# USTC3DV/D3Human-code

Measured on AMD Instinct MI355X. Metric: train iters/sec @ tet-res 128, 1024^2 render; 1/2/4/8 MI355X, higher is better.
Workload: dtype f32

## Files before the change

d3human-code_amd/csrc/sdf_mlp_bwd.hip:

```cpp
#include "sdf_mlp_dev.h"
#include "sdf_mlp_x3.h"
#include <type_traits>

using namespace D3H_MLP_NS;

namespace {

__global__ void sdf_mlp_pack_t_kernel(const float* __restrict__ w0, const float* __restrict__ wh, const float* __restrict__ w4,
                                      float* __restrict__ wpackT) {
    int idx = blockIdx.x * blockDim.x + threadIdx.x;
    if (idx >= WPACKT_FLOATS) return;
    int l = t_layer_of_offset(idx);
    int local = idx - t_layer_offset(l);
    int r = local & 3, lane = (local >> 2) & 63, rest = local >> 8;
    int i = lane & 15, q = lane >> 4;
    int blk = rest & 15, rbg = rest >> 4;
    int out = 16 * blk + 4 * q + r;
    int in = 16 * rbg + i;
    float v = 0.f;
    if (l == 0) {
        if (in < EMB_DIM) v = w0[out * EMB_DIM + in];
    } else if (l == 4) {
        if (rbg < 16) v = w4[out * (256 + EMB_DIM) + in];
        else {
            int e = in - 256;
            if (e < EMB_DIM) v = w4[out * (256 + EMB_DIM) + 256 + e];
        }
    } else {
        int hi = (l < 4) ? (l - 1) : (l - 2);
        v = wh[(size_t)hi * 65536 + out * 256 + in];
    }
    wpackT[idx] = v;
}

__global__ __launch_bounds__(256) void sdf_mlp_active_tiles_kernel(const float* __restrict__ gout, int64_t n, int ntiles16, int* __restrict__ list,
                                                                   int* __restrict__ count) {
    int t = blockIdx.x * 256 + threadIdx.x;
    bool act = false;
    if (t < ntiles16) {
        int64_t p0 = (int64_t)t * 16;
#pragma unroll
        for (int k = 0; k < 16; ++k)
            if (p0 + k < n) {
#pragma unroll
                for (int o = 0; o < NOUT; ++o)
                    if (gout[(p0 + k) * NOUT + o] != 0.f) act = true;
            }
    }
    unsigned long long m = __ballot(act);
    int lane = threadIdx.x & 63;
    int base = 0;
    if (lane == 0 && m) base = atomicAdd(count, __popcll(m));
    base = __shfl(base, 0);
    if (act) list[base + __popcll(m & ((1ull << lane) - 1ull))] = t;
}

#if D3H_MLP_NOUT == 1
__global__ __launch_bounds__(256) void sdf_mlp_active_points_kernel(const float* __restrict__ gout, int64_t n, int* __restrict__ plist, int* __restrict__ counts) {
    const int64_t p = (int64_t)blockIdx.x * 256 + threadIdx.x;
    const float gv = p < n ? gout[p] : 0.f;
    const bool act = p < n && gv != 0.f;
    {
        float m = fabsf(gv);
        if (!(m < 3.0e38f)) m = 0.f;
#pragma unroll
        for (int k = 32; k > 0; k >>= 1) m = fmaxf(m, __shfl_xor(m, k));
        if ((threadIdx.x & 63) == 0 && m > 0.f) atomicMax((unsigned*)counts + 2, __float_as_uint(m));
    }
    const unsigned long long m = __ballot(act);
    const int lane = threadIdx.x & 63;
    int base = 0;
    if (lane == 0 && m) base = atomicAdd(counts, __popcll(m));
    base = __shfl(base, 0);
    if (act) plist[base + __popcll(m & ((1ull << lane) - 1ull))] = (int)p;
}
__global__ __launch_bounds__(256) void sdf_mlp_gather_points_kernel(const float* __restrict__ x, const float* __restrict__ deform, float disp,
                                                                    const float* __restrict__ gout, const int* __restrict__ plist, int* __restrict__ counts,
                                                                    int* __restrict__ ident, float* __restrict__ xg, float* __restrict__ gg) {
    const int cnt = counts[0];
    const int ntile = (cnt + 15) >> 4;
    if (blockIdx.x == 0 && threadIdx.x == 0) counts[1] = ntile;
    for (int g = blockIdx.x * 256 + threadIdx.x; g < ntile * 16; g += gridDim.x * 256) {
        float x0 = 0.f, x1 = 0.f, x2 = 0.f, gv = 0.f;
        if (g < cnt) {
            const int64_t p = plist[g];
            x0 = x[3 * p + 0]; x1 = x[3 * p + 1]; x2 = x[3 * p + 2];
            if (deform) {
                x0 = __fadd_rn(x0, __fmul_rn(disp, deform[3 * p + 0]));
                x1 = __fadd_rn(x1, __fmul_rn(disp, deform[3 * p + 1]));
                x2 = __fadd_rn(x2, __fmul_rn(disp, deform[3 * p + 2]));
            }
            gv = gout[p];
        }
        xg[3 * (size_t)g + 0] = x0; xg[3 * (size_t)g + 1] = x1; xg[3 * (size_t)g + 2] = x2;
        gg[g] = gv;
        if ((g & 15) == 0) ident[g >> 4] = g >> 4;
    }
}
__global__ __launch_bounds__(256) void sdf_mlp_gather_gout_kernel(const float* __restrict__ gout, const int* __restrict__ plist, int* __restrict__ counts,
                                                                  float* __restrict__ gg) {
    const int cnt = counts[0];
    const int ntile = (cnt + 15) >> 4;
    float m = 0.f;
    for (int g = blockIdx.x * 256 + threadIdx.x; g < ntile * 16; g += gridDim.x * 256) {
        const float gv = g < cnt ? gout[plist[g]] : 0.f;
        gg[g] = gv;
        const float a = fabsf(gv);
        if (a < 3.0e38f) m = fmaxf(m, a);
    }
#pragma unroll
    for (int k = 32; k > 0; k >>= 1) m = fmaxf(m, __shfl_xor(m, k));
    if ((threadIdx.x & 63) == 0 && m > 0.f) atomicMax((unsigned*)counts + 6, __float_as_uint(m));
}
__global__ __launch_bounds__(256) void sdf_mlp_scatter_dx_kernel(const float* __restrict__ dxg, const int* __restrict__ plist, const int* __restrict__ counts,
                                                                 float* __restrict__ dx) {
    const int cnt = counts[0];
    for (int g = blockIdx.x * 256 + threadIdx.x; g < cnt; g += gridDim.x * 256) {
        const int64_t p = plist[g];
        dx[3 * p + 0] = dxg[3 * (size_t)g + 0]; dx[3 * p + 1] = dxg[3 * (size_t)g + 1]; dx[3 * p + 2] = dxg[3 * (size_t)g + 2];
    }
}
#endif

__device__ __forceinline__ void dz_block(f32x4& v, const float* act_l, float* dz_l, int rb, int lane) {
    size_t off = (size_t)(rb * 64 + lane) * 4;
    f32x4 hh = *(const f32x4*)(act_l + off);
    f32x4 o;
#pragma unroll
    for (int r = 0; r < 4; ++r) {
        o[r] = v[r] * dsoftplus_from_h(hh[r]);
        v[r] = o[r];
    }
    *(f32x4*)(dz_l + off) = o;
}

__device__ __forceinline__ void dz_block_inject(f32x4& v, const float* act_l, float* e_l, int rb, int lane) {
    size_t off = (size_t)(rb * 64 + lane) * 4;
    f32x4 hh = *(const f32x4*)(act_l + off);
    f32x4 ee = *(const f32x4*)(e_l + off);
    f32x4 o;
#pragma unroll
    for (int r = 0; r < 4; ++r) {
        o[r] = v[r] * dsoftplus_from_h(hh[r]) + ee[r];
        v[r] = o[r];
    }
    *(f32x4*)(e_l + off) = o;
}

__device__ __forceinline__ void dz_block_pre(f32x4& v, const f32x4 hh, float* dz_l, int rb, int lane) {
    f32x4 o;
#pragma unroll
    for (int r = 0; r < 4; ++r) {
        o[r] = v[r] * dsoftplus_from_h(hh[r]);
        v[r] = o[r];
    }
    *(f32x4*)(dz_l + (size_t)(rb * 64 + lane) * 4) = o;
}
__device__ __forceinline__ void dz_block_inject_pre(f32x4& v, const f32x4 hh, const f32x4 ee, float* e_l, int rb, int lane) {
    f32x4 o;
#pragma unroll
    for (int r = 0; r < 4; ++r) {
        o[r] = v[r] * dsoftplus_from_h(hh[r]) + ee[r];
        v[r] = o[r];
    }
    *(f32x4*)(e_l + (size_t)(rb * 64 + lane) * 4) = o;
}


template <bool INJECT>
__global__ __launch_bounds__(NTHREADS, 2) void sdf_mlp_bwd_data_kernel(const float* __restrict__ x, const float* __restrict__ deform, float disp,
                                                                      const float* __restrict__ gout, const float* __restrict__ w7,
                                                                      const float* __restrict__ wpackT, const float* __restrict__ act,
                                                                      float* __restrict__ dz, float* __restrict__ dx, int64_t n, int ntiles,
                                                                      const int* __restrict__ tile_list, const int* __restrict__ tile_count) {
    __shared__ __attribute__((aligned(16))) float wbuf[2][T_CHUNK_FLOATS];
    __shared__ __attribute__((aligned(16))) float w7s[NOUT * 256];
    __shared__ __attribute__((aligned(16))) float pfb[NWAVES * (INJECT ? 4 : 2) * 256];
    const int n_active = tile_list ? *tile_count : 0;
    const int64_t n16 = tile_list ? (int64_t)n_active : (int64_t)ntiles * 8;
    const int G = (int)gridDim.x;
    const int nrounds = (int)((n16 + NWAVES * (int64_t)G - 1) / (NWAVES * (int64_t)G));

    const int tid = threadIdx.x;
    const int lane = tid & 63;
    const int wave = tid >> 6;
    const int q = lane >> 4;
    constexpr int N4 = T_CHUNK_FLOATS / 4;

    for (int j = tid; j < NOUT * 256; j += NTHREADS) w7s[j] = w7[j];
    Stage st;
    int pb = 0;
    SDF_STAGE_ISSUE(st, wpackT, wbuf[0], N4, tid);
    SDF_STAGE_COMMIT(st, wbuf[0], N4, tid);

    f32x4 X[16], Y[16];
#if D3H_SDF_PRIO
    if (wave >= 4) __builtin_amdgcn_s_setprio(1);
#endif

    for (int rnd = 0; rnd < nrounds; ++rnd) {
        const int64_t seq = (int64_t)rnd * NWAVES * G + (int64_t)wave * G + blockIdx.x;
        const bool on = seq < n16;
        const int64_t t16 = on ? (tile_list ? (int64_t)tile_list[seq] : seq) : 0;
        const int64_t p = t16 * 16 + (lane & 15);
        const bool valid = on && p < n;
        const float* act_tile = act + t16 * ACT_TILE_FLOATS;
        float* dz_tile = dz + t16 * ACT_TILE_FLOATS;
        float g[NOUT];
#pragma unroll
        for (int o = 0; o < NOUT; ++o) g[o] = INJECT ? 0.f : (valid ? (gout ? gout[p * NOUT + o] : 1.f) : 0.f);

#pragma unroll
        for (int rb = 0; rb < 16; ++rb) {
            X[rb] = (f32x4){0.f, 0.f, 0.f, 0.f};
#pragma unroll
            for (int o = 0; o < NOUT; ++o) {
                f32x4 w = *(const f32x4*)(w7s + 256 * o + 16 * rb + 4 * q);
#pragma unroll
                for (int r = 0; r < 4; ++r) X[rb][r] = fmaf(g[o], w[r], X[rb][r]);
            }
        }

        f32x4 E[EMB_BLKS];
#pragma unroll
        for (int b = 0; b < EMB_BLKS; ++b) E[b] = (f32x4){0.f, 0.f, 0.f, 0.f};

        float* pf = pfb + wave * ((INJECT ? 4 : 2) * 256);
        auto prefetch = [&](int lp, int c) {
            const size_t o0 = (size_t)lp * ACT_LAYER_FLOATS + (size_t)((2 * c) * 64 + lane) * 4;
            D3H_GLDS16(act_tile + o0, pf);
            D3H_GLDS16(act_tile + o0 + 256, pf + 256);
            if (INJECT) {
                D3H_GLDS16(dz_tile + o0, pf + 512);
                D3H_GLDS16(dz_tile + o0 + 256, pf + 768);
            }
        };
        auto dz_pair = [&](f32x4& v0, f32x4& v1, int lp, int c) {
            const float* pl = pf + lane * 4;
            float* dzl = dz_tile + lp * ACT_LAYER_FLOATS;
            if (INJECT) {
                dz_block_inject_pre(v0, *(const f32x4*)pl, *(const f32x4*)(pl + 512), dzl, 2 * c, lane);
                dz_block_inject_pre(v1, *(const f32x4*)(pl + 256), *(const f32x4*)(pl + 768), dzl, 2 * c + 1, lane);
            } else {
                dz_block_pre(v0, *(const f32x4*)pl, dzl, 2 * c, lane);
                dz_block_pre(v1, *(const f32x4*)(pl + 256), dzl, 2 * c + 1, lane);
            }
        };
        const float* next = wpackT + T_CHUNK_FLOATS;
        for (int it = 0; it < 3; ++it) {
            {
                const int l = 6 - 2 * it;
                if (on && it == 0) {
#pragma unroll
                    for (int rb = 0; rb < 16; ++rb) {
                        if (INJECT) dz_block_inject(X[rb], act_tile + l * ACT_LAYER_FLOATS, dz_tile + l * ACT_LAYER_FLOATS, rb, lane);
                        else dz_block(X[rb], act_tile + l * ACT_LAYER_FLOATS, dz_tile + l * ACT_LAYER_FLOATS, rb, lane);
                    }
                }
#pragma unroll
                for (int c = 0; c < 8; ++c) {
                    SDF_STAGE_ISSUE(st, next, wbuf[pb ^ 1], N4, tid);
                    next += T_CHUNK_FLOATS;
                    if (on) prefetch(l - 1, c);
                    if (on) {
                        f32x4 acc0 = {0.f, 0.f, 0.f, 0.f}, acc1 = {0.f, 0.f, 0.f, 0.f};
                        mac_hidden2(acc0, acc1, X, wbuf[pb], 16 * 256, lane);
                        Y[2 * c] = acc0;
                        Y[2 * c + 1] = acc1;
                    }
                    __builtin_amdgcn_s_waitcnt(0x0f70);
                    SDF_STAGE_COMMIT(st, wbuf[pb ^ 1], N4, tid);
                    pb ^= 1;
                    if (on) dz_pair(Y[2 * c], Y[2 * c + 1], l - 1, c);
                }
                if (l == 4) {
#pragma unroll
                    for (int c = 0; c < 2; ++c) {
                        SDF_STAGE_ISSUE(st, next, wbuf[pb ^ 1], N4, tid);
                        next += T_CHUNK_FLOATS;
                        if (on) {
                            mac_hidden(E[2 * c], X, wbuf[pb], lane);
                            if (2 * c + 1 < EMB_BLKS) mac_hidden(E[2 * c + 1], X, wbuf[pb] + 16 * 256, lane);
                        }
                        SDF_STAGE_COMMIT(st, wbuf[pb ^ 1], N4, tid);
                        pb ^= 1;
                    }
                }
            }
            {
                const int l = 5 - 2 * it;
#pragma unroll
                for (int c = 0; c < 8; ++c) {
                    SDF_STAGE_ISSUE(st, next, wbuf[pb ^ 1], N4, tid);
                    next += T_CHUNK_FLOATS;
                    if (on) prefetch(l - 1, c);
                    if (on) {
                        f32x4 acc0 = {0.f, 0.f, 0.f, 0.f}, acc1 = {0.f, 0.f, 0.f, 0.f};
                        mac_hidden2(acc0, acc1, Y, wbuf[pb], 16 * 256, lane);
                        X[2 * c] = acc0;
                        X[2 * c + 1] = acc1;
                    }
                    __builtin_amdgcn_s_waitcnt(0x0f70);
                    SDF_STAGE_COMMIT(st, wbuf[pb ^ 1], N4, tid);
                    pb ^= 1;
                    if (on) dz_pair(X[2 * c], X[2 * c + 1], l - 1, c);
                }
            }
        }
#pragma unroll
        for (int c = 0; c < 2; ++c) {
            SDF_STAGE_ISSUE(st, (c == 0) ? next : wpackT, wbuf[pb ^ 1], N4, tid);
            next += T_CHUNK_FLOATS;
            if (on) {
                mac_hidden(E[2 * c], X, wbuf[pb], lane);
                if (2 * c + 1 < EMB_BLKS) mac_hidden(E[2 * c + 1], X, wbuf[pb] + 16 * 256, lane);
            }
            SDF_STAGE_COMMIT(st, wbuf[pb ^ 1], N4, tid);
            pb ^= 1;
        }

        if (!INJECT && dx && on) {
            float x0 = 0.f, x1 = 0.f, x2 = 0.f;
            if (valid) {
                x0 = x[3 * p + 0]; x1 = x[3 * p + 1]; x2 = x[3 * p + 2];
                if (deform) {
                    x0 = __fadd_rn(x0, __fmul_rn(disp, deform[3 * p + 0]));
                    x1 = __fadd_rn(x1, __fmul_rn(disp, deform[3 * p + 1]));
                    x2 = __fadd_rn(x2, __fmul_rn(disp, deform[3 * p + 2]));
                }
            }
            float d0 = 0.f, d1 = 0.f, d2 = 0.f;
#pragma unroll
            for (int b = 0; b < EMB_BLKS; ++b)
#pragma unroll
                for (int r = 0; r < 4; ++r) {
                    int e = 16 * b + 4 * q + r;
                    if (e < EMB_DIM) {
                        float ge = E[b][r];
                        int c;
                        float coef;
                        if (e < 3) { c = e; coef = 1.f; }
                        else {
                            int ep = e - 3;
                            int fr = ep / 6, fn = (ep % 6) / 3;
                            c = ep % 3;
                            float f = (float)(1 << fr);
                            float xc = c == 0 ? x0 : (c == 1 ? x1 : x2);
                            coef = fn ? (-f * sinf(f * xc)) : (f * cosf(f * xc));
                        }
                        float t = ge * coef;
                        if (c == 0) d0 += t; else if (c == 1) d1 += t; else d2 += t;
                    }
                }
            d0 += __shfl_xor(d0, 16); d0 += __shfl_xor(d0, 32);
            d1 += __shfl_xor(d1, 16); d1 += __shfl_xor(d1, 32);
            d2 += __shfl_xor(d2, 16); d2 += __shfl_xor(d2, 32);
            if (valid && q == 0) { dx[3 * p + 0] = d0; dx[3 * p + 1] = d1; dx[3 * p + 2] = d2; }
        }
    }
#if D3H_SDF_GLDS
    __builtin_amdgcn_s_waitcnt(0x0f70);
#endif
}

#if D3H_MLP_NOUT == 1
template <int NP>
__global__ void sdf_mlp_pack_t3_kernel(const float* __restrict__ w0, const float* __restrict__ wh, const float* __restrict__ w4,
                                       unsigned* __restrict__ wpackT3) {
    int idx = blockIdx.x * blockDim.x + threadIdx.x;
    if (idx >= XPT<NP>::WPACKT_DWORDS) return;
    const int chunk = idx / XPT<NP>::HID_CHUNK;
    const int l = t_layer_of_offset(chunk * T_CHUNK_FLOATS);
    const int local = idx - (t_layer_offset(l) / T_CHUNK_FLOATS) * XPT<NP>::HID_CHUNK;
    const int d = local & 3, lane = (local >> 2) & 63;
    int rest = local >> 8;
    const int part = rest % NP;
    rest /= NP;
    const int kb = rest & 7, rbg = rest >> 3;
    const int i = lane & 15, q = lane >> 4;
    const int in = 16 * rbg + i;
    unsigned bits[2];
#pragma unroll
    for (int e = 0; e < 2; ++e) {
        const int out = x3_feature(kb, q, 2 * d + e);
        float v = 0.f;
        if (l == 0) {
            if (in < EMB_DIM) v = w0[out * EMB_DIM + in];
        } else if (l == 4) {
            if (rbg < 16) v = w4[out * (256 + EMB_DIM) + in];
            else if (in - 256 < EMB_DIM) v = w4[out * (256 + EMB_DIM) + in];
        } else {
            const int hi = (l < 4) ? (l - 1) : (l - 2);
            v = wh[(size_t)hi * 65536 + out * 256 + in];
        }
        unsigned h, m, lo = 0;
        if constexpr (NP == 3) x3_split_pair(v, 0.f, h, m, lo);
        else {
            h2_split_pair(v, 0.f, h, m);
            if (!(fabsf(v) <= 16384.0f)) h = m = 0x7e00u;
        }
        bits[e] = (part == 0 ? h : (part == 1 ? m : lo)) & 0xffffu;
    }
    wpackT3[idx] = bits[0] | (bits[1] << 16);
}

__global__ __launch_bounds__(256) void h2_scale_from_absmax_kernel(const float* __restrict__ v, int64_t n, const unsigned* __restrict__ bits, float* __restrict__ sc) {
    __shared__ float red[256];
    float m = 0.f;
    if (bits) m = __uint_as_float(*bits);
    else
        for (int64_t i = threadIdx.x; i < n; i += 256) m = fmaxf(m, fabsf(v[i]));
    red[threadIdx.x] = m;
    __syncthreads();
    for (int k = 128; k > 0; k >>= 1) {
        if ((int)threadIdx.x < k) red[threadIdx.x] = fmaxf(red[threadIdx.x], red[threadIdx.x + k]);
        __syncthreads();
    }
    if (threadIdx.x == 0) {
        const float s = h2_grad_scale(red[0]);
        sc[0] = s;
        sc[1] = 1.0f / s;
    }
}

template <bool SCALED>
__device__ __forceinline__ void dzs_plain(f32x4& v, const f32x4 hh, float* dz_l, int rb, int lane, float gsi) {
    f32x4 o;
#pragma unroll
    for (int r = 0; r < 4; ++r) {
        v[r] = v[r] * dsoftplus_from_h(hh[r]);
        o[r] = SCALED ? v[r] * gsi : v[r];
    }
    *(f32x4*)(dz_l + (size_t)(rb * 64 + lane) * 4) = o;
}
template <bool SCALED>
__device__ __forceinline__ void dzs_inject(f32x4& v, const f32x4 hh, const f32x4 ee, float* e_l, int rb, int lane, float gs, float gsi) {
    f32x4 o;
#pragma unroll
    for (int r = 0; r < 4; ++r) {
        v[r] = SCALED ? fmaf(ee[r], gs, v[r] * dsoftplus_from_h(hh[r])) : (v[r] * dsoftplus_from_h(hh[r]) + ee[r]);
        o[r] = SCALED ? v[r] * gsi : v[r];
    }
    *(f32x4*)(e_l + (size_t)(rb * 64 + lane) * 4) = o;
}

template <bool INJECT, int NP>
__global__ __launch_bounds__(NTHREADS, 2) void sdf_mlp_bwd_data_x3_kernel(const float* __restrict__ x, const float* __restrict__ deform, float disp,
                                                                         const float* __restrict__ gout, const float* __restrict__ w7,
                                                                         const unsigned* __restrict__ wpackT3, const float* __restrict__ act,
                                                                         float* __restrict__ dz, float* __restrict__ dx, int64_t n, int ntiles,
                                                                         const int* __restrict__ tile_list, const int* __restrict__ tile_count,
                                                                         const float* __restrict__ sc_dev, float sc_imm) {
    constexpr int X3_HID_CHUNK = XPT<NP>::HID_CHUNK;
    const float gs = (NP == 2) ? (sc_dev ? sc_dev[0] : sc_imm) : 1.0f;
    const float gsi = (NP == 2) ? (sc_dev ? sc_dev[1] : 1.0f / sc_imm) : 1.0f;
    __shared__ __attribute__((aligned(16))) unsigned wbuf[2][X3_HID_CHUNK];
    __shared__ __attribute__((aligned(16))) float w7s[NOUT * 256];
    __shared__ __attribute__((aligned(16))) float pfb[NWAVES * (INJECT ? 4 : 2) * 256];
    D3H_X3_CLAIM_SIMD();
    const int n_active = tile_list ? *tile_count : 0;
    const int64_t n16 = tile_list ? (int64_t)n_active : (int64_t)ntiles * 8;
    const int G = (int)gridDim.x;
    const int nrounds = (int)((n16 + NWAVES * (int64_t)G - 1) / (NWAVES * (int64_t)G));

    const int tid = threadIdx.x;
    const int lane = tid & 63;
    const int wave = __builtin_amdgcn_readfirstlane(tid >> 6);
    const int q = lane >> 4;
    constexpr int N4 = X3_HID_CHUNK / 4;
    constexpr int RS = 8 * NP * X3_FRAG;

    for (int j = tid; j < NOUT * 256; j += NTHREADS) w7s[j] = w7[j];
    int pb = 0;
    x3_issue(wpackT3, wbuf[0], N4, tid);
    glds_commit();

    u32x4 Xs[8][NP];
    f32x4 Y[16];

    for (int rnd = 0; rnd < nrounds; ++rnd) {
        const int64_t seq = (int64_t)rnd * NWAVES * G + (int64_t)wave * G + blockIdx.x;
        const bool on = seq < n16;
        const int64_t t16 = on ? (tile_list ? (int64_t)tile_list[seq] : seq) : 0;
        const int64_t p = t16 * 16 + (lane & 15);
        const bool valid = on && p < n;
        const float* act_tile = act + t16 * ACT_TILE_FLOATS;
        float* dz_tile = dz + t16 * ACT_TILE_FLOATS;
        float g[NOUT];
#pragma unroll
        for (int o = 0; o < NOUT; ++o) g[o] = INJECT ? 0.f : (valid ? (gout ? gout[p * NOUT + o] : 1.f) * gs : 0.f);

#pragma unroll
        for (int rb = 0; rb < 16; ++rb) {
            Y[rb] = (f32x4){0.f, 0.f, 0.f, 0.f};
#pragma unroll
            for (int o = 0; o < NOUT; ++o) {
                f32x4 w = *(const f32x4*)(w7s + 256 * o + 16 * rb + 4 * q);
#pragma unroll
                for (int r = 0; r < 4; ++r) Y[rb][r] = fmaf(g[o], w[r], Y[rb][r]);
            }
            if (on) {
                const size_t off6 = (size_t)6 * ACT_LAYER_FLOATS + (size_t)(rb * 64 + lane) * 4;
                const f32x4 hh6 = *(const f32x4*)(act_tile + off6);
                if (INJECT) dzs_inject<NP == 2>(Y[rb], hh6, *(const f32x4*)(dz_tile + off6), dz_tile + 6 * ACT_LAYER_FLOATS, rb, lane, gs, gsi);
                else dzs_plain<NP == 2>(Y[rb], hh6, dz_tile + 6 * ACT_LAYER_FLOATS, rb, lane, gsi);
            }
        }
#pragma unroll
        for (int kb = 0; kb < 8; ++kb) xp_split_blocks<NP>(Y[2 * kb], Y[2 * kb + 1], Xs[kb]);

        f32x4 E[4], Elo[4];
#pragma unroll
        for (int b = 0; b < 4; ++b) E[b] = Elo[b] = (f32x4){0.f, 0.f, 0.f, 0.f};

        float* pf = pfb + wave * ((INJECT ? 4 : 2) * 256);
        auto prefetch = [&](int lp, int c) {
            const size_t o0 = (size_t)lp * ACT_LAYER_FLOATS + (size_t)((2 * c) * 64 + lane) * 4;
            D3H_GLDS16(act_tile + o0, pf);
            D3H_GLDS16(act_tile + o0 + 256, pf + 256);
            if (INJECT) {
                D3H_GLDS16(dz_tile + o0, pf + 512);
                D3H_GLDS16(dz_tile + o0 + 256, pf + 768);
            }
        };
        auto dz_pair = [&](f32x4& v0, f32x4& v1, int lp, int c) {
            const float* pl = pf + lane * 4;
            float* dzl = dz_tile + lp * ACT_LAYER_FLOATS;
            if (INJECT) {
                dzs_inject<NP == 2>(v0, *(const f32x4*)pl, *(const f32x4*)(pl + 512), dzl, 2 * c, lane, gs, gsi);
                dzs_inject<NP == 2>(v1, *(const f32x4*)(pl + 256), *(const f32x4*)(pl + 768), dzl, 2 * c + 1, lane, gs, gsi);
            } else {
                dzs_plain<NP == 2>(v0, *(const f32x4*)pl, dzl, 2 * c, lane, gsi);
                dzs_plain<NP == 2>(v1, *(const f32x4*)(pl + 256), dzl, 2 * c + 1, lane, gsi);
            }
        };
        auto emb_chunks = [&](const unsigned* last) {
#pragma unroll
            for (int c = 0; c < 2; ++c) {
                x3_issue(c == 0 ? last : last + X3_HID_CHUNK, wbuf[pb ^ 1], N4, tid);
                if (on) {
                    xp_mac_blocks<NP, 8, -1>(E[2 * c], Elo[2 * c], Xs, wbuf[pb], lane, X3None());
                    if (2 * c + 1 < EMB_BLKS) xp_mac_blocks<NP, 8, -1>(E[2 * c + 1], Elo[2 * c + 1], Xs, wbuf[pb] + RS, lane, X3None());
                }
                glds_commit();
                pb ^= 1;
            }
        };
        const unsigned* next = wpackT3 + X3_HID_CHUNK;
#pragma unroll 1
        for (int l = 6; l >= 1; --l) {
#pragma unroll
            for (int c = 0; c < 8; ++c) {
                x3_issue(next, wbuf[pb ^ 1], N4, tid);
                next += X3_HID_CHUNK;
                if (on) {
                    prefetch(l - 1, c);
                    f32x4 acc0 = {0.f, 0.f, 0.f, 0.f}, acc1 = {0.f, 0.f, 0.f, 0.f}, lo0 = {0.f, 0.f, 0.f, 0.f}, lo1 = {0.f, 0.f, 0.f, 0.f};
                    xp_mac_blocks<NP, 8, -1>(acc0, lo0, Xs, wbuf[pb], lane, X3None());
                    xp_mac_blocks<NP, 8, -1>(acc1, lo1, Xs, wbuf[pb] + RS, lane, X3None());
                    Y[2 * c] = xp_fold<NP>(acc0, lo0);
                    Y[2 * c + 1] = xp_fold<NP>(acc1, lo1);
                }
                glds_commit();
                pb ^= 1;
                if (on) dz_pair(Y[2 * c], Y[2 * c + 1], l - 1, c);
            }
            if (l == 4) {
                emb_chunks(next);
                next += 2 * X3_HID_CHUNK;
            }
#pragma unroll
            for (int kb = 0; kb < 8; ++kb) xp_split_blocks<NP>(Y[2 * kb], Y[2 * kb + 1], Xs[kb]);
        }
#pragma unroll
        for (int c = 0; c < 2; ++c) {
            x3_issue((c == 0) ? next : wpackT3, wbuf[pb ^ 1], N4, tid);
            if (on) {
                xp_mac_blocks<NP, 8, -1>(E[2 * c], Elo[2 * c], Xs, wbuf[pb], lane, X3None());
                if (2 * c + 1 < EMB_BLKS) xp_mac_blocks<NP, 8, -1>(E[2 * c + 1], Elo[2 * c + 1], Xs, wbuf[pb] + RS, lane, X3None());
            }
            glds_commit();
            pb ^= 1;
        }
#pragma unroll
        for (int b = 0; b < 4; ++b) E[b] = xp_fold<NP>(E[b], Elo[b]);

        if (!INJECT && dx && on) {
            float x0 = 0.f, x1 = 0.f, x2 = 0.f;
            if (valid) {
                x0 = x[3 * p + 0]; x1 = x[3 * p + 1]; x2 = x[3 * p + 2];
                if (deform) {
                    x0 = __fadd_rn(x0, __fmul_rn(disp, deform[3 * p + 0]));
                    x1 = __fadd_rn(x1, __fmul_rn(disp, deform[3 * p + 1]));
                    x2 = __fadd_rn(x2, __fmul_rn(disp, deform[3 * p + 2]));
                }
            }
            float d0 = 0.f, d1 = 0.f, d2 = 0.f;
#pragma unroll
            for (int b = 0; b < EMB_BLKS; ++b)
#pragma unroll
                for (int r = 0; r < 4; ++r) {
                    int e = 16 * b + 4 * q + r;
                    if (e < EMB_DIM) {
                        float ge = E[b][r];
                        int c;
                        float coef;
                        if (e < 3) { c = e; coef = 1.f; }
                        else {
                            int ep = e - 3;
                            int fr = ep / 6, fn = (ep % 6) / 3;
                            c = ep % 3;
                            float f = (float)(1 << fr);
                            float xc = c == 0 ? x0 : (c == 1 ? x1 : x2);
                            coef = fn ? (-f * sinf(f * xc)) : (f * cosf(f * xc));
                        }
                        float t = ge * coef;
                        if (c == 0) d0 += t; else if (c == 1) d1 += t; else d2 += t;
                    }
                }
            d0 += __shfl_xor(d0, 16); d0 += __shfl_xor(d0, 32);
            d1 += __shfl_xor(d1, 16); d1 += __shfl_xor(d1, 32);
            d2 += __shfl_xor(d2, 16); d2 += __shfl_xor(d2, 32);
            if (valid && q == 0) { dx[3 * p + 0] = d0 * gsi; dx[3 * p + 1] = d1 * gsi; dx[3 * p + 2] = d2 * gsi; }
        }
    }
    __builtin_amdgcn_s_waitcnt(0x0f70);
}
template <bool INJECT>
static inline void bwd_data_x_launch(int planes, int grid, hipStream_t s, const float* x, const float* deform, float disp, const float* gout, const float* w7,
                                     const unsigned* wpackT, const float* act, float* dz, float* dx, int64_t n, int ntiles, const int* list, const int* cnt,
                                     const float* sc_dev, float sc_imm) {
    if (planes == 2)
        hipLaunchKernelGGL((sdf_mlp_bwd_data_x3_kernel<INJECT, 2>), dim3(grid), dim3(NTHREADS), 0, s, x, deform, disp, gout, w7, wpackT, act, dz, dx, n, ntiles,
                           list, cnt, sc_dev, sc_imm);
    else
        hipLaunchKernelGGL((sdf_mlp_bwd_data_x3_kernel<INJECT, 3>), dim3(grid), dim3(NTHREADS), 0, s, x, deform, disp, gout, w7, wpackT, act, dz, dx, n, ntiles,
                           list, cnt, (const float*)nullptr, 1.0f);
}
#endif

constexpr int PITCH = 33;

constexpr int LAST_UNROLL = 4, LAST_GRID = 128;
#ifndef D3H_DW_SPLIT
#define D3H_DW_SPLIT 128
#endif
constexpr int DW_SPLIT = D3H_DW_SPLIT;
#ifndef D3H_DW_SPLIT_EMB
#define D3H_DW_SPLIT_EMB 128
#endif
#ifndef D3H_DW_SPLIT_SPARSE
#define D3H_DW_SPLIT_SPARSE 32
#endif
static inline bool dw_h2_enabled() {
    static int v = -1;
    if (v < 0) { const char* e = getenv("D3H_DW_H2"); v = (e && e[0] == '0') ? 0 : 1; }
    return v == 1;
}
static inline bool dw_x3_enabled(int which) {
    static int v = -1;
    if (v < 0) {
        const char* e = getenv("D3H_DW_X3");
        v = e ? atoi(e) : 1;
    }
    return v == 1 || v == which;
}
static inline int dw_split(int nt32, int cap) {
    int s = nt32 / 8;
    if (s < 16) s = 16;
    if (s > cap) s = cap;
    if (s > nt32) s = nt32;
    return s < 1 ? 1 : s;
}
template <int NCB, bool EMB>
__device__ __forceinline__ void sdf_mlp_bwd_dw_body(const float* __restrict__ dz_l , const float* __restrict__ hsrc ,
                                                    const float* __restrict__ x, const float* __restrict__ deform, float disp,
                                                    int64_t n, int ntiles32, float* __restrict__ dW, int ld, int coloff,
                                                    int ncols, float* __restrict__ db, const float* __restrict__ udir,
                                                    const int* __restrict__ tile_list, const int* __restrict__ tile_count,
                                                    const float* __restrict__ dz2, const float* __restrict__ hsrc2) {
    __shared__ float TA[256 * PITCH];
    __shared__ float TB[NCB * 32 * PITCH];

    const int tid = threadIdx.x;
    const int lane = tid & 63, wave = tid >> 6;
    const int i = lane & 31, h = lane >> 5;
    const int rg = wave & 3;
    const int cg = wave >> 2;
    constexpr int CBW = NCB / 2;
    const int cchunk = blockIdx.y;

    f32x16 acc[2][CBW];
#pragma unroll
    for (int a = 0; a < 2; ++a)
#pragma unroll
        for (int b = 0; b < CBW; ++b) acc[a][b] = (f32x16){0};
    float dbsum = 0.f;

    const int n_active = tile_list ? *tile_count : 0;
    if (tile_list) ntiles32 = (n_active + 1) >> 1;
    auto tile_of = [&](int g16) -> int64_t { return tile_list ? (g16 < n_active ? (int64_t)tile_list[g16] : (int64_t)-1) : (int64_t)g16; };
    const f32x4 zero4 = {0.f, 0.f, 0.f, 0.f};

    f32x4 ra[4], rb_[NCB / 2];
    float re[4];
    const int ngroups = dz2 ? 2 * ntiles32 : ntiles32;
    auto issue = [&](int tv) {
        const bool second = dz2 && tv >= ntiles32;
        const int t = second ? tv - ntiles32 : tv;
        const float* __restrict__ asrc = second ? dz2 : dz_l;
        const float* __restrict__ bsrc = second ? hsrc2 : hsrc;
        const float* __restrict__ ud = second ? nullptr : udir;
#pragma unroll
        for (int r = 0; r < 4; ++r) {
            int u = tid + 512 * r;
            int t2 = u >> 10, rem = u & 1023;
            int64_t tl = tile_of(2 * t + t2);
            ra[r] = tl >= 0 ? *(const f32x4*)(asrc + (size_t)tl * ACT_TILE_FLOATS + 4 * (size_t)rem) : zero4;
        }
        if (EMB) {
#pragma unroll
            for (int r = 0; r < 4; ++r) {
                int u = tid + 512 * r;
                int e = u >> 5, pt = u & 31;
                int64_t tl = tile_of(2 * t + (pt >> 4));
                int64_t p = tl * 16 + (pt & 15);
                float v = 0.f;
                if (tl >= 0 && p < n && e < EMB_DIM) {
                    float x0 = x[3 * p + 0], x1 = x[3 * p + 1], x2 = x[3 * p + 2];
                    if (deform) {
                        x0 = __fadd_rn(x0, __fmul_rn(disp, deform[3 * p + 0]));
                        x1 = __fadd_rn(x1, __fmul_rn(disp, deform[3 * p + 1]));
                        x2 = __fadd_rn(x2, __fmul_rn(disp, deform[3 * p + 2]));
                    }
                    v = ud ? emb_tangent(e, x0, x1, x2, ud[3 * p + 0], ud[3 * p + 1], ud[3 * p + 2]) : emb_feature(e, x0, x1, x2);
                }
                re[r] = v;
            }
        } else {
            const int rb0 = cchunk * NCB * 2;
#pragma unroll
            for (int r = 0; r < NCB / 2; ++r) {
                int u = tid + 512 * r;
                int t2 = u / (NCB * 128), rem = u % (NCB * 128);
                int rbl = rem >> 6, ln = rem & 63;
                int64_t tl = tile_of(2 * t + t2);
                rb_[r] = tl >= 0 ? *(const f32x4*)(bsrc + (size_t)tl * ACT_TILE_FLOATS + 4 * (size_t)((rb0 + rbl) * 64 + ln)) : zero4;
            }
        }
    };
    auto commit = [&]() {
#pragma unroll
        for (int r = 0; r < 4; ++r) {
            int u = tid + 512 * r;
            int t2 = u >> 10, rem = u & 1023;
            int ln = rem & 63, rbk = rem >> 6;
            int f = 16 * rbk + 4 * (ln >> 4), pt = 16 * t2 + (ln & 15);
#pragma unroll
            for (int k = 0; k < 4; ++k) TA[(f + k) * PITCH + pt] = ra[r][k];
        }
        if (EMB) {
#pragma unroll
            for (int r = 0; r < 4; ++r) {
                int u = tid + 512 * r;
                TB[(u >> 5) * PITCH + (u & 31)] = re[r];
            }
        } else {
#pragma unroll
            for (int r = 0; r < NCB / 2; ++r) {
                int u = tid + 512 * r;
                int t2 = u / (NCB * 128), rem = u % (NCB * 128);
                int rbl = rem >> 6, ln = rem & 63;
                int f = 16 * rbl + 4 * (ln >> 4), pt = 16 * t2 + (ln & 15);
#pragma unroll
                for (int k = 0; k < 4; ++k) TB[(f + k) * PITCH + pt] = rb_[r][k];
            }
        }
    };
    int t = blockIdx.x;
    if (t >= ngroups) return;
    issue(t);
    for (; t < ngroups; t += gridDim.x) {
        commit();
        __syncthreads();
        if (t + (int)gridDim.x < ngroups) issue(t + gridDim.x);
#pragma unroll 4
        for (int s = 0; s < 16; ++s) {
            float a0 = TA[((rg * 2 + 0) * 32 + i) * PITCH + 2 * s + h];
            float a1 = TA[((rg * 2 + 1) * 32 + i) * PITCH + 2 * s + h];
#pragma unroll
            for (int b = 0; b < CBW; ++b) {
                float bv = TB[((cg * CBW + b) * 32 + i) * PITCH + 2 * s + h];
                acc[0][b] = __builtin_amdgcn_mfma_f32_32x32x2f32(a0, bv, acc[0][b], 0, 0, 0);
                acc[1][b] = __builtin_amdgcn_mfma_f32_32x32x2f32(a1, bv, acc[1][b], 0, 0, 0);
            }
        }
        if (db && cchunk == 0 && tid < 256 && (!dz2 || t >= ntiles32)) {
            float sm = 0.f;
#pragma unroll 8
            for (int pt = 0; pt < 32; ++pt) sm += TA[tid * PITCH + pt];
            dbsum += sm;
        }
        __syncthreads();
    }
#pragma unroll
    for (int a = 0; a < 2; ++a)
#pragma unroll
        for (int b = 0; b < CBW; ++b) {
            int col = cchunk * NCB * 32 + (cg * CBW + b) * 32 + i;
            if (col < ncols) {
#pragma unroll
                for (int r = 0; r < 16; ++r) {
                    int row = (rg * 2 + a) * 32 + (r & 3) + 8 * (r >> 2) + 4 * h;
                    atomicAdd(&dW[(size_t)row * ld + coloff + col], acc[a][b][r]);
#ifdef D3H_DW_DOUBLEFLUSH
                    atomicAdd(&dW[(size_t)row * ld + coloff + col], acc[a][b][r] * 0.f);
#endif
                }
            }
        }
    if (db && cchunk == 0 && tid < 256) atomicAdd(&db[tid], dbsum);
}

struct DwEmbArgs {
    const float* dz_l; const float* hsrc; float* dW; int ld, coloff, ncols; float* db; const float* udir; const float* dz2; const float* hsrc2;
};
__global__ __launch_bounds__(512) void sdf_mlp_bwd_dw_emb_pair_kernel(DwEmbArgs a0, DwEmbArgs a1, const float* __restrict__ x, const float* __restrict__ deform,
                                                                       float disp, int64_t n, int ntiles32, const int* __restrict__ tile_list,
                                                                       const int* __restrict__ tile_count) {
    const DwEmbArgs a = blockIdx.z ? a1 : a0;
    sdf_mlp_bwd_dw_body<2, true>(a.dz_l, a.hsrc, x, deform, disp, n, ntiles32, a.dW, a.ld, a.coloff, a.ncols, a.db, a.udir, tile_list, tile_count, a.dz2,
                                 a.hsrc2);
}

template <int NCB, bool EMB>
__global__ __launch_bounds__(512) void sdf_mlp_bwd_dw_kernel(const float* __restrict__ dz_l, const float* __restrict__ hsrc, const float* __restrict__ x,
                                                             const float* __restrict__ deform, float disp, int64_t n, int ntiles32,
                                                             float* __restrict__ dW, int ld, int coloff, int ncols, float* __restrict__ db,
                                                             const float* __restrict__ udir, const int* __restrict__ tile_list,
                                                             const int* __restrict__ tile_count, const float* __restrict__ dz2,
                                                             const float* __restrict__ hsrc2) {
    sdf_mlp_bwd_dw_body<NCB, EMB>(dz_l, hsrc, x, deform, disp, n, ntiles32, dW, ld, coloff, ncols, db, udir, tile_list, tile_count, dz2, hsrc2);
}

__global__ __launch_bounds__(512) void sdf_mlp_bwd_dw_layers_kernel(const float* __restrict__ a_base, const float* __restrict__ b_base,
                                                                    const float* __restrict__ x, int64_t n, int ntiles32,
                                                                    float* __restrict__ dwh, float* __restrict__ dbh, float* __restrict__ dw4,
                                                                    float* __restrict__ db4, const int* __restrict__ tile_list,
                                                                    const int* __restrict__ tile_count, const float* __restrict__ a2_base,
                                                                    const float* __restrict__ b2_base) {
    const int l = blockIdx.z + 1;
    const int hi = (l < 4) ? (l - 1) : (l - 2);
    float* dW = (l == 4) ? dw4 : dwh + (size_t)hi * 65536;
    float* db = (l == 4) ? db4 : dbh + hi * 256;
    const int ld = (l == 4) ? 256 + EMB_DIM : 256;
    sdf_mlp_bwd_dw_body<4, false>(a_base + (size_t)l * ACT_LAYER_FLOATS, b_base + (size_t)(l - 1) * ACT_LAYER_FLOATS, x, nullptr, 0.f, n, ntiles32,
                                  dW, ld, 0, 256, db, nullptr, tile_list, tile_count,
                                  a2_base ? a2_base + (size_t)l * ACT_LAYER_FLOATS : nullptr,
                                  b2_base ? b2_base + (size_t)(l - 1) * ACT_LAYER_FLOATS : nullptr);
}

#if D3H_MLP_NOUT == 1
constexpr int DWX_PITCH = 12;
#ifndef D3H_EMULATED
#define D3H_MFMA32_BF16X8(a, b, c) \
    __builtin_amdgcn_mfma_f32_32x32x16_bf16(__builtin_bit_cast(d3h_bf16x8, a), __builtin_bit_cast(d3h_bf16x8, b), c, 0, 0, 0)
#define D3H_MFMA32_F16X8(a, b, c) \
    __builtin_amdgcn_mfma_f32_32x32x16_f16(__builtin_bit_cast(d3h_f16x8, a), __builtin_bit_cast(d3h_f16x8, b), c, 0, 0, 0)
#else
#define D3H_MFMA32_BF16X8(a, b, c) emul::mfma_32x32x16bf16(a, b, c)
#define D3H_MFMA32_F16X8(a, b, c) emul::mfma_32x32x16f16(a, b, c)
#endif

__device__ __forceinline__ void dwx_put(unsigned* T, int nrows, int f0, int j, const f32x4 v) {
    const bool odd = j & 1;
    const float ma = odd ? v[2] : v[0], mb = odd ? v[3] : v[1];
    const float xa = __shfl_xor(odd ? v[0] : v[2], 1), xb = __shfl_xor(odd ? v[1] : v[3], 1);
    const int f = f0 + (odd ? 2 : 0), w = j >> 1;
    unsigned h, m, lo;
    x3_split_pair(odd ? xa : ma, odd ? ma : xa, h, m, lo);
    T[(0 * nrows + f) * DWX_PITCH + w] = h;
    T[(1 * nrows + f) * DWX_PITCH + w] = m;
    T[(2 * nrows + f) * DWX_PITCH + w] = lo;
    x3_split_pair(odd ? xb : mb, odd ? mb : xb, h, m, lo);
    T[(0 * nrows + f + 1) * DWX_PITCH + w] = h;
    T[(1 * nrows + f + 1) * DWX_PITCH + w] = m;
    T[(2 * nrows + f + 1) * DWX_PITCH + w] = lo;
}

__global__ __launch_bounds__(512) void sdf_mlp_bwd_dw_layers_x3_kernel(const float* __restrict__ a_base, const float* __restrict__ b_base, int ntiles16,
                                                                       float* __restrict__ dwh, float* __restrict__ dbh, float* __restrict__ dw4,
                                                                       float* __restrict__ db4, const int* __restrict__ tile_list,
                                                                       const int* __restrict__ tile_count, const float* __restrict__ a2_base,
                                                                       const float* __restrict__ b2_base) {
    constexpr int NP = 3;
#ifndef D3H_DWX_PIPE
#define D3H_DWX_PIPE 0
#endif
    constexpr int NIMG = D3H_DWX_PIPE ? 2 : 1;
    __shared__ __attribute__((aligned(16))) unsigned TA3s[NIMG][NP * 256 * DWX_PITCH];
    __shared__ __attribute__((aligned(16))) unsigned TB3s[NIMG][NP * 128 * DWX_PITCH];
    unsigned* TA3 = TA3s[0];
    unsigned* TB3 = TB3s[0];
#ifdef D3H_DWX_PROBE_LDSPAD
    __shared__ volatile unsigned ldspad[D3H_DWX_PROBE_LDSPAD / 4];
    ldspad[threadIdx.x * 16 % (D3H_DWX_PROBE_LDSPAD / 4)] = threadIdx.x;
#endif
    D3H_X3_CLAIM_SIMD();
    const int l = blockIdx.z + 1;
    const int hi = (l < 4) ? (l - 1) : (l - 2);
    float* dW = (l == 4) ? dw4 : dwh + (size_t)hi * 65536;
    float* db = (l == 4) ? db4 : dbh + hi * 256;
    const int ld = (l == 4) ? 256 + EMB_DIM : 256;
    const float* dz_l = a_base + (size_t)l * ACT_LAYER_FLOATS;
    const float* hsrc = b_base + (size_t)(l - 1) * ACT_LAYER_FLOATS;
    const float* dz2 = a2_base ? a2_base + (size_t)l * ACT_LAYER_FLOATS : nullptr;
    const float* hsrc2 = b2_base ? b2_base + (size_t)(l - 1) * ACT_LAYER_FLOATS : nullptr;

    const int tid = threadIdx.x;
    const int lane = tid & 63, wave = __builtin_amdgcn_readfirstlane(tid >> 6);
    const int i = lane & 31, h = lane >> 5;
    const int rg = wave & 3, cg = wave >> 2;
    const int cchunk = blockIdx.y;
    const bool want_db = cchunk == 0 && cg == 0;

    f32x16 acc[2][2], accdb[2];
#pragma unroll
    for (int a = 0; a < 2; ++a) {
        accdb[a] = (f32x16){0};
#pragma unroll
        for (int b = 0; b < 2; ++b) acc[a][b] = (f32x16){0};
    }
    const int n16 = tile_list ? *tile_count : ntiles16;
    const int ngroups = dz2 ? 2 * n16 : n16;

    f32x4 ra[2], rbv;
    auto issue = [&](int tv) {
        const bool second = dz2 && tv >= n16;
        const int t = second ? tv - n16 : tv;
        const int64_t tl = tile_list ? (int64_t)tile_list[t] : (int64_t)t;
        const float* __restrict__ asrc = (second ? dz2 : dz_l) + (size_t)tl * ACT_TILE_FLOATS;
        const float* __restrict__ bsrc = (second ? hsrc2 : hsrc) + (size_t)tl * ACT_TILE_FLOATS;
        ra[0] = *(const f32x4*)(asrc + 4 * (size_t)tid);
        ra[1] = *(const f32x4*)(asrc + 4 * (size_t)(tid + 512));
        rbv = *(const f32x4*)(bsrc + 4 * (size_t)(cchunk * 512 + tid));
    };
    int t = blockIdx.x;
    if (t >= ngroups) return;
    const u32x4 ones = {0x3f803f80u, 0x3f803f80u, 0x3f803f80u, 0x3f803f80u};
    issue(t);
#ifdef D3H_DWX_PROBE_NOWORK
    t = ngroups;
#endif
#if D3H_DWX_PIPE && !defined(D3H_EMULATED)
    {
        int cur = 0;
        dwx_put(TA3s[0], 256, 16 * wave + 4 * (lane >> 4), lane & 15, ra[0]);
        dwx_put(TA3s[0], 256, 16 * (wave + 8) + 4 * (lane >> 4), lane & 15, ra[1]);
        dwx_put(TB3s[0], 128, 16 * wave + 4 * (lane >> 4), lane & 15, rbv);
        __syncthreads();
        if (t + (int)gridDim.x < ngroups) issue(t + gridDim.x);
        for (; t < ngroups; t += gridDim.x) {
            const bool bias_now = want_db && db && (!dz2 || t >= n16);
            const bool more = t + (int)gridDim.x < ngroups;
            const unsigned* TAc = TA3s[cur];
            const unsigned* TBc = TB3s[cur];
            u32x4 A[2][3], B[2][3];
#pragma unroll
            for (int a = 0; a < 2; ++a)
#pragma unroll
                for (int pl = 0; pl < 3; ++pl) {
                    A[a][pl] = *(const u32x4*)(TAc + (pl * 256 + (rg * 2 + a) * 32 + i) * DWX_PITCH + 4 * h);
                    B[a][pl] = *(const u32x4*)(TBc + (pl * 128 + (cg * 2 + a) * 32 + i) * DWX_PITCH + 4 * h);
                }
            auto body = [&](auto with_bias) {
                dwx_put(TA3s[cur ^ 1], 256, 16 * wave + 4 * (lane >> 4), lane & 15, ra[0]);
                dwx_put(TA3s[cur ^ 1], 256, 16 * (wave + 8) + 4 * (lane >> 4), lane & 15, ra[1]);
                dwx_put(TB3s[cur ^ 1], 128, 16 * wave + 4 * (lane >> 4), lane & 15, rbv);
#pragma unroll
                for (int a = 0; a < 2; ++a) {
#pragma unroll
                    for (int b = 0; b < 2; ++b) {
                        f32x16 c = acc[a][b];
                        c = D3H_MFMA32_BF16X8(A[a][2], B[b][0], c);
                        c = D3H_MFMA32_BF16X8(A[a][0], B[b][2], c);
                        c = D3H_MFMA32_BF16X8(A[a][1], B[b][1], c);
                        c = D3H_MFMA32_BF16X8(A[a][1], B[b][0], c);
                        c = D3H_MFMA32_BF16X8(A[a][0], B[b][1], c);
                        c = D3H_MFMA32_BF16X8(A[a][0], B[b][0], c);
                        acc[a][b] = c;
                    }
                    if (decltype(with_bias)::value) {
                        accdb[a] = D3H_MFMA32_BF16X8(A[a][2], ones, accdb[a]);
                        accdb[a] = D3H_MFMA32_BF16X8(A[a][1], ones, accdb[a]);
                        accdb[a] = D3H_MFMA32_BF16X8(A[a][0], ones, accdb[a]);
                    }
                }
#pragma unroll
                for (int k = 0; k < (decltype(with_bias)::value ? 30 : 24); ++k) {
                    __builtin_amdgcn_sched_group_barrier(0x008, 1, 0);
                    __builtin_amdgcn_sched_group_barrier(0x002, 5, 0);
                    __builtin_amdgcn_sched_group_barrier(0x200, 1, 0);
                }
            };
            (void)more;
            if (bias_now) body(std::true_type{}); else body(std::false_type{});
            __syncthreads();
            if (t + 2 * (int)gridDim.x < ngroups) issue(t + 2 * gridDim.x);
            cur ^= 1;
        }
    }
#else
    for (; t < ngroups; t += gridDim.x) {
#ifndef D3H_DWX_PROBE_NOPUT
        dwx_put(TA3, 256, 16 * wave + 4 * (lane >> 4), lane & 15, ra[0]);
        dwx_put(TA3, 256, 16 * (wave + 8) + 4 * (lane >> 4), lane & 15, ra[1]);
        dwx_put(TB3, 128, 16 * wave + 4 * (lane >> 4), lane & 15, rbv);
#endif
        const bool bias_now = want_db && db && (!dz2 || t >= n16);
        __syncthreads();
        if (t + (int)gridDim.x < ngroups) issue(t + gridDim.x);
        u32x4 A[2][NP], B[2][NP];
#pragma unroll
        for (int a = 0; a < 2; ++a)
#pragma unroll
            for (int pl = 0; pl < NP; ++pl) {
                A[a][pl] = *(const u32x4*)(TA3 + (pl * 256 + (rg * 2 + a) * 32 + i) * DWX_PITCH + 4 * h);
                B[a][pl] = *(const u32x4*)(TB3 + (pl * 128 + (cg * 2 + a) * 32 + i) * DWX_PITCH + 4 * h);
            }
#ifdef D3H_DWX_PROBE_NOMFMA
        acc[0][0][0] += __uint_as_float(A[0][0][0] ^ B[0][0][0] ^ A[1][NP - 1][3] ^ B[1][NP - 1][3]) * 0.f;
#else
#pragma unroll
        for (int a = 0; a < 2; ++a) {
#pragma unroll
            for (int b = 0; b < 2; ++b) {
                f32x16 c = acc[a][b];
                c = D3H_MFMA32_BF16X8(A[a][2], B[b][0], c);
                c = D3H_MFMA32_BF16X8(A[a][0], B[b][2], c);
                c = D3H_MFMA32_BF16X8(A[a][1], B[b][1], c);
                c = D3H_MFMA32_BF16X8(A[a][1], B[b][0], c);
                c = D3H_MFMA32_BF16X8(A[a][0], B[b][1], c);
                c = D3H_MFMA32_BF16X8(A[a][0], B[b][0], c);
                acc[a][b] = c;
            }
            if (bias_now) {
                accdb[a] = D3H_MFMA32_BF16X8(A[a][2], ones, accdb[a]);
                accdb[a] = D3H_MFMA32_BF16X8(A[a][1], ones, accdb[a]);
                accdb[a] = D3H_MFMA32_BF16X8(A[a][0], ones, accdb[a]);
            }
        }
#endif
        __syncthreads();
    }
#endif
#ifdef D3H_DWX_PROBE_NOFLUSH
    if (acc[0][0][0] != 12345.678f) return;
#endif
#pragma unroll
    for (int a = 0; a < 2; ++a) {
#pragma unroll
        for (int b = 0; b < 2; ++b) {
            const int col = cchunk * 128 + (cg * 2 + b) * 32 + i;
#pragma unroll
            for (int r = 0; r < 16; ++r) {
                const int row = (rg * 2 + a) * 32 + (r & 3) + 8 * (r >> 2) + 4 * h;
                atomicAdd(&dW[(size_t)row * ld + col], acc[a][b][r]);
            }
        }
        if (want_db && db && i == 0) {
#pragma unroll
            for (int r = 0; r < 16; ++r) atomicAdd(&db[(rg * 2 + a) * 32 + (r & 3) + 8 * (r >> 2) + 4 * h], accdb[a][r]);
        }
    }
}

constexpr float DWH_US = 64.0f;
__device__ __forceinline__ void dwh_split_pair(float a, float b, unsigned& h, unsigned& m) {
    h = h2_pk(a, b);
    m = h2_pk(a - h2_lo(h), b - h2_hi(h));
}
__device__ __forceinline__ void dwh_put(unsigned* T, int nrows, int f0, int j, f32x4 v, float sc) {
#pragma unroll
    for (int r = 0; r < 4; ++r) v[r] *= sc;
    const bool odd = j & 1;
    const float ma = odd ? v[2] : v[0], mb = odd ? v[3] : v[1];
    const float xa = __shfl_xor(odd ? v[0] : v[2], 1), xb = __shfl_xor(odd ? v[1] : v[3], 1);
    const int f = f0 + (odd ? 2 : 0), w = j >> 1;
    unsigned h, m;
    dwh_split_pair(odd ? xa : ma, odd ? ma : xa, h, m);
    T[(0 * nrows + f) * DWX_PITCH + w] = h;
    T[(1 * nrows + f) * DWX_PITCH + w] = m;
    dwh_split_pair(odd ? xb : mb, odd ? mb : xb, h, m);
    T[(0 * nrows + f + 1) * DWX_PITCH + w] = h;
    T[(1 * nrows + f + 1) * DWX_PITCH + w] = m;
}

__global__ __launch_bounds__(512) void sdf_mlp_bwd_dw_layers_h2_kernel(const float* __restrict__ a_base, const float* __restrict__ b_base, int ntiles16,
                                                                       float* __restrict__ dwh, float* __restrict__ dbh, float* __restrict__ dw4,
                                                                       float* __restrict__ db4, const int* __restrict__ tile_list,
                                                                       const int* __restrict__ tile_count, const float* __restrict__ a2_base,
                                                                       const float* __restrict__ b2_base, const float* __restrict__ sc_dev, float sc_imm,
                                                                       int sc_mask) {
    __shared__ __attribute__((aligned(16))) unsigned TAs[2][2 * 256 * DWX_PITCH];
    __shared__ __attribute__((aligned(16))) unsigned TBs[2][2 * 128 * DWX_PITCH];
    D3H_X3_CLAIM_SIMD();
    const float gs = sc_dev ? sc_dev[0] : sc_imm;
    const float gsi = sc_dev ? sc_dev[1] : 1.0f / sc_imm;
    const int l = blockIdx.z + 1;
    const int hi = (l < 4) ? (l - 1) : (l - 2);
    float* dW = (l == 4) ? dw4 : dwh + (size_t)hi * 65536;
    float* db = (l == 4) ? db4 : dbh + hi * 256;
    const int ld = (l == 4) ? 256 + EMB_DIM : 256;
    const float* dz_l = a_base + (size_t)l * ACT_LAYER_FLOATS;
    const float* hsrc = b_base + (size_t)(l - 1) * ACT_LAYER_FLOATS;
    const float* dz2 = a2_base ? a2_base + (size_t)l * ACT_LAYER_FLOATS : nullptr;
    const float* hsrc2 = b2_base ? b2_base + (size_t)(l - 1) * ACT_LAYER_FLOATS : nullptr;

    const int tid = threadIdx.x;
    const int lane = tid & 63, wave = __builtin_amdgcn_readfirstlane(tid >> 6);
    const int i = lane & 31, h = lane >> 5;
    const int rg = wave & 3, cg = wave >> 2;
    const int cchunk = blockIdx.y;
    const bool want_db = cchunk == 0 && cg == 0;

    f32x16 acc[2][2], accdb[2];
#pragma unroll
    for (int a = 0; a < 2; ++a) {
        accdb[a] = (f32x16){0};
#pragma unroll
        for (int b = 0; b < 2; ++b) acc[a][b] = (f32x16){0};
    }
    const int n16 = tile_list ? *tile_count : ntiles16;
    const int ngroups = dz2 ? 2 * n16 : n16;
    const int G2 = 2 * (int)gridDim.x;
    int t = 2 * (int)blockIdx.x;
    if (t >= ngroups) return;

    f32x4 ra[2][2], rb[2];
    float sca[2], scb[2];
    auto issue = [&](int slot, int tv) {
        const bool second = dz2 && tv >= n16;
        const int tt = second ? tv - n16 : tv;
        const int64_t tl = tile_list ? (int64_t)tile_list[tt] : (int64_t)tt;
        const float* __restrict__ asrc = (second ? dz2 : dz_l) + (size_t)tl * ACT_TILE_FLOATS;
        const float* __restrict__ bsrc = (second ? hsrc2 : hsrc) + (size_t)tl * ACT_TILE_FLOATS;
        ra[slot][0] = *(const f32x4*)(asrc + 4 * (size_t)tid);
        ra[slot][1] = *(const f32x4*)(asrc + 4 * (size_t)(tid + 512));
        rb[slot] = *(const f32x4*)(bsrc + 4 * (size_t)(cchunk * 512 + tid));
        sca[slot] = ((sc_mask >> (second ? 2 : 0)) & 1) ? gs : DWH_US;
        scb[slot] = ((sc_mask >> (second ? 3 : 1)) & 1) ? gs : DWH_US;
    };
    const u32x4 ones = {0x3c003c00u, 0x3c003c00u, 0x3c003c00u, 0x3c003c00u};
    issue(0, t);
    if (t + 1 < ngroups) issue(1, t + 1);
    for (; t < ngroups; t += G2) {
        const bool two = t + 1 < ngroups;
#pragma unroll
        for (int sl = 0; sl < 2; ++sl) {
            if (sl == 1 && !two) break;
            dwh_put(TAs[sl], 256, 16 * wave + 4 * (lane >> 4), lane & 15, ra[sl][0], sca[sl]);
            dwh_put(TAs[sl], 256, 16 * (wave + 8) + 4 * (lane >> 4), lane & 15, ra[sl][1], sca[sl]);
            dwh_put(TBs[sl], 128, 16 * wave + 4 * (lane >> 4), lane & 15, rb[sl], scb[sl]);
        }
        const bool bias0 = want_db && db && (!dz2 || t >= n16);
        const bool bias1 = want_db && db && two && (!dz2 || t + 1 >= n16);
        __syncthreads();
        if (t + G2 < ngroups) {
            issue(0, t + G2);
            if (t + G2 + 1 < ngroups) issue(1, t + G2 + 1);
        }
#pragma unroll
        for (int sl = 0; sl < 2; ++sl) {
            if (sl == 1 && !two) break;
            u32x4 A[2][2], B[2][2];
#pragma unroll
            for (int a = 0; a < 2; ++a)
#pragma unroll
                for (int pl = 0; pl < 2; ++pl) {
                    A[a][pl] = *(const u32x4*)(TAs[sl] + (pl * 256 + (rg * 2 + a) * 32 + i) * DWX_PITCH + 4 * h);
                    B[a][pl] = *(const u32x4*)(TBs[sl] + (pl * 128 + (cg * 2 + a) * 32 + i) * DWX_PITCH + 4 * h);
                }
            const bool bias_now = sl == 0 ? bias0 : bias1;
#pragma unroll
            for (int a = 0; a < 2; ++a) {
#pragma unroll
                for (int b = 0; b < 2; ++b) {
                    f32x16 c = acc[a][b];
                    c = D3H_MFMA32_F16X8(A[a][1], B[b][0], c);
                    c = D3H_MFMA32_F16X8(A[a][0], B[b][1], c);
                    c = D3H_MFMA32_F16X8(A[a][0], B[b][0], c);
                    acc[a][b] = c;
                }
                if (bias_now) {
                    accdb[a] = D3H_MFMA32_F16X8(A[a][1], ones, accdb[a]);
                    accdb[a] = D3H_MFMA32_F16X8(A[a][0], ones, accdb[a]);
                }
            }
        }
        __syncthreads();
    }
    const float wsc = gsi * (1.0f / DWH_US);
    const bool a_flag = dz2 ? ((sc_mask >> 2) & 1) : (sc_mask & 1);
    const float bsc = a_flag ? gsi : (1.0f / DWH_US);
#pragma unroll
    for (int a = 0; a < 2; ++a) {
#pragma unroll
        for (int b = 0; b < 2; ++b) {
            const int col = cchunk * 128 + (cg * 2 + b) * 32 + i;
#pragma unroll
            for (int r = 0; r < 16; ++r) {
                const int row = (rg * 2 + a) * 32 + (r & 3) + 8 * (r >> 2) + 4 * h;
                atomicAdd(&dW[(size_t)row * ld + col], acc[a][b][r] * wsc);
            }
        }
        if (want_db && db && i == 0) {
#pragma unroll
            for (int r = 0; r < 16; ++r) atomicAdd(&db[(rg * 2 + a) * 32 + (r & 3) + 8 * (r >> 2) + 4 * h], accdb[a][r] * bsc);
        }
    }
}
#endif

__global__ __launch_bounds__(256) void sdf_mlp_bwd_last_kernel(const float* __restrict__ gout, const float* __restrict__ act6, int64_t n,
                                                               int ntiles16, float* __restrict__ dW7, float* __restrict__ db7,
                                                               const int* __restrict__ tile_list, const int* __restrict__ tile_count) {
    const int tid = threadIdx.x, lane = tid & 63, wave = tid >> 6;
    if (tile_list) ntiles16 = *tile_count;
    const int q = lane >> 4;
    const int o = blockIdx.y;
    dW7 += 256 * o;
    if (db7) db7 += o;
    f32x4 part[4];
#pragma unroll
    for (int a = 0; a < 4; ++a) part[a] = (f32x4){0.f, 0.f, 0.f, 0.f};
    float gsum = 0.f;
    for (int ti0 = blockIdx.x * LAST_UNROLL; ti0 < ntiles16; ti0 += gridDim.x * LAST_UNROLL) {
        float g[LAST_UNROLL];
        f32x4 hh[LAST_UNROLL][4];
#pragma unroll
        for (int u = 0; u < LAST_UNROLL; ++u) {
            const int ti = ti0 + u;
            const bool live = ti < ntiles16;
            const int64_t t = live ? (tile_list ? (int64_t)tile_list[ti] : (int64_t)ti) : 0;
            int64_t p = t * 16 + (lane & 15);
            g[u] = (live && p < n) ? (gout ? gout[p * NOUT + o] : 1.f) : 0.f;
            const float* base = act6 + (size_t)t * ACT_TILE_FLOATS;
#pragma unroll
            for (int a = 0; a < 4; ++a)
                hh[u][a] = live ? *(const f32x4*)(base + (size_t)((wave + 4 * a) * 64 + lane) * 4) : (f32x4){0.f, 0.f, 0.f, 0.f};
        }
#pragma unroll
        for (int u = 0; u < LAST_UNROLL; ++u) {
            if (wave == 0 && q == 0) gsum += g[u];
#pragma unroll
            for (int a = 0; a < 4; ++a)
#pragma unroll
                for (int k = 0; k < 4; ++k) part[a][k] = fmaf(g[u], hh[u][a][k], part[a][k]);
        }
    }
#pragma unroll
    for (int a = 0; a < 4; ++a)
#pragma unroll
        for (int k = 0; k < 4; ++k) {
            float v = part[a][k];
            for (int m = 8; m >= 1; m >>= 1) v += __shfl_xor(v, m);
            if ((lane & 15) == 0) atomicAdd(&dW7[16 * (wave + 4 * a) + 4 * q + k], v);
        }
    for (int m = 8; m >= 1; m >>= 1) gsum += __shfl_xor(gsum, m);
    if (tid == 0 && db7) atomicAdd(db7, gsum);
}

#if D3H_MLP_NOUT == 1
__global__ __launch_bounds__(256) void eikonal_loss_kernel(const float* __restrict__ g, int64_t n, float scale, float* __restrict__ loss_sum,
                                                           float* __restrict__ u) {
    __shared__ float s4[4];
    float acc = 0.f;
    for (int64_t i = (int64_t)blockIdx.x * 256 + threadIdx.x; i < n; i += (int64_t)gridDim.x * 256) {
        float a = g[3 * i], b = g[3 * i + 1], c = g[3 * i + 2];
        float nrm = sqrtf(a * a + b * b + c * c);
        float d = nrm - 1.0f;
        acc += d * d;
        if (u) {
            float k = scale * 2.0f * d / nrm;
            u[3 * i] = k * a; u[3 * i + 1] = k * b; u[3 * i + 2] = k * c;
        }
    }
    for (int m = 32; m >= 1; m >>= 1) acc += __shfl_xor(acc, m);
    if ((threadIdx.x & 63) == 0) s4[threadIdx.x >> 6] = acc;
    __syncthreads();
    if (threadIdx.x == 0) atomicAdd(loss_sum, s4[0] + s4[1] + s4[2] + s4[3]);
}

#endif

}

#if D3H_MLP_NOUT == 1
int d3h_sdf_mlp_fwd_x3_list_launch(const float* x, const float* deform, float disp, const unsigned* wpack3, int planes, float* act, int64_t n,
                                   const int* tile_list, const int* tile_count, hipStream_t s);
extern "C" int d3h_sdf_mlp_fwd_x3(const float* x, const float* deform, float disp, const unsigned* wpack3, float* sdf, float* xdef, float* act,
                                  int64_t n, int max_cus, void* stream);
extern "C" int d3h_sdf_mlp_fwd_h2(const float* x, const float* deform, float disp, const unsigned* wpackh2, float* sdf, float* xdef, float* act,
                                  int64_t n, int max_cus, void* stream);
#endif
static inline int64_t bwd_r4(int64_t v) { return (v + 3) & ~(int64_t)3; }
static inline int64_t bwd_p16(int64_t n) { return (n + 15) & ~(int64_t)15; }

extern "C" int64_t d3h_sdf_mlp_bwd_scratch_ints(int64_t n) { return 8 + bwd_r4(n) + bwd_r4(n / 16 + 2) + 7 * bwd_p16(n) + 64; }

extern "C" int64_t d3h_sdf_mlp_wpackt_floats(void) { return WPACKT_FLOATS; }

extern "C" int d3h_sdf_mlp_pack_t(const float* w0, const float* wh, const float* w4, float* wpackT, void* stream) {
    if (!w0 || !wh || !w4 || !wpackT) return D3H_ERR_ARG;
    hipLaunchKernelGGL(sdf_mlp_pack_t_kernel, dim3(d3h_cdiv(WPACKT_FLOATS, 256)), dim3(256), 0, (hipStream_t)stream, w0, wh, w4, wpackT);
    D3H_LAUNCH_CHECK();
    return D3H_OK;
}

#if D3H_MLP_NOUT == 1
extern "C" int64_t d3h_sdf_mlp_wpackt3_dwords(void) { return X3_WPACKT_DWORDS; }

extern "C" int d3h_sdf_mlp_pack_t3(const float* w0, const float* wh, const float* w4, unsigned* wpackT3, void* stream) {
    if (!w0 || !wh || !w4 || !wpackT3) return D3H_ERR_ARG;
    hipLaunchKernelGGL(sdf_mlp_pack_t3_kernel<3>, dim3(d3h_cdiv(X3_WPACKT_DWORDS, 256)), dim3(256), 0, (hipStream_t)stream, w0, wh, w4, wpackT3);
    D3H_LAUNCH_CHECK();
    return D3H_OK;
}

extern "C" int64_t d3h_sdf_mlp_wpackth2_dwords(void) { return XPT<2>::WPACKT_DWORDS; }

extern "C" int d3h_sdf_mlp_pack_t_h2(const float* w0, const float* wh, const float* w4, unsigned* wpackTh2, void* stream) {
    if (!w0 || !wh || !w4 || !wpackTh2) return D3H_ERR_ARG;
    hipLaunchKernelGGL(sdf_mlp_pack_t3_kernel<2>, dim3(d3h_cdiv(XPT<2>::WPACKT_DWORDS, 256)), dim3(256), 0, (hipStream_t)stream, w0, wh, w4, wpackTh2);
    D3H_LAUNCH_CHECK();
    return D3H_OK;
}
#endif

#if D3H_MLP_NOUT == 1
extern "C" int d3h_sdf_mlp_bwd_prepare(const float* x, const float* deform, float disp, const float* marks, int64_t n, int* tile_list,
                                       const unsigned* wpack3_recompute, int recompute_planes, float* act, void* stream) {
    if (n < 0 || n >= (int64_t)1 << 31 || !x || !marks || !tile_list || !wpack3_recompute || !act || (recompute_planes != 2 && recompute_planes != 3)) return D3H_ERR_ARG;
    if (n == 0) return D3H_OK;
    hipStream_t s = (hipStream_t)stream;
    int* counts = tile_list;
    int* pl = counts + 8;
    int* ident = pl + bwd_r4(n);
    float* xg = (float*)(ident + bwd_r4(n / 16 + 2));
    float* gg = xg + 3 * bwd_p16(n);
    (void)hipMemsetAsync(counts, 0, 8 * sizeof(int), s);
    hipLaunchKernelGGL(sdf_mlp_active_points_kernel, dim3((unsigned)d3h_cdiv(n, 256)), dim3(256), 0, s, marks, n, pl, counts);
    hipLaunchKernelGGL(sdf_mlp_gather_points_kernel, dim3(256), dim3(256), 0, s, x, deform, disp, marks, (const int*)pl, counts, ident, xg, gg);
    int e = d3h_sdf_mlp_fwd_x3_list_launch(xg, nullptr, 0.f, wpack3_recompute, recompute_planes, act, n, ident, counts + 1, s);
    if (e != 0) return e;
    D3H_LAUNCH_CHECK();
    return D3H_OK;
}
#endif

extern "C" int d3h_sdf_mlp_bwd(const float* x, const float* deform, float disp, const float* gout, const float* w7,
                               const float* wpackT, const unsigned* wpackT3, const float* act, float* dz, int64_t n, float* dx, float* dw0, float* db0,
                               float* dwh, float* dbh, float* dw4, float* db4, float* dw7, float* db7, int* tile_list,
                               const unsigned* wpack3_recompute, int recompute_planes, int t_planes, int prepared, void* stream) {
    if (n < 0) return D3H_ERR_ARG;
    if (prepared && !(tile_list && wpack3_recompute)) return D3H_ERR_ARG;
    if (wpack3_recompute && recompute_planes != 2 && recompute_planes != 3) return D3H_ERR_ARG;
    if (wpackT3 && t_planes != 2 && t_planes != 3) return D3H_ERR_ARG;
    const float* sc_dev = nullptr;
    float* sc_tmp = nullptr;
    if (n == 0) return D3H_OK;
    if (!x || !gout || !w7 || (!wpackT && !wpackT3) || !act || !dz || !dw0 || !db0 || !dwh || !dbh || !dw4 || !db4 || !dw7 || !db7) return D3H_ERR_ARG;
    hipStream_t s = (hipStream_t)stream;
    int ntiles = (int)((n + TILE_PTS - 1) / TILE_PTS);
    int nt32 = ntiles * 4;
    int nt16 = ntiles * 8;
    int grid = sdf_chain_grid(ntiles, 0);
    const int* list = nullptr;
    const int* cnt = nullptr;
    const float *xs = x, *dfs = deform, *gs = gout;
    float disps = disp, *dxs = dx;
    const int* plist = nullptr;
    const int* pcounts = nullptr;
#if D3H_MLP_NOUT == 1
    if (wpack3_recompute && !wpackT3) return D3H_ERR_ARG;
    if (tile_list && wpack3_recompute) {
        if (n >= (int64_t)1 << 31) return D3H_ERR_ARG;
        int* counts = tile_list;
        int* pl = counts + 8;
        int* ident = pl + bwd_r4(n);
        float* xg = (float*)(ident + bwd_r4(n / 16 + 2));
        float* gg = xg + 3 * bwd_p16(n);
        float* dxg = gg + bwd_p16(n);
        if (dx) (void)hipMemsetAsync(dx, 0, (size_t)n * 3 * sizeof(float), s);
        if (prepared) {
            hipLaunchKernelGGL(sdf_mlp_gather_gout_kernel, dim3(64), dim3(256), 0, s, gout, (const int*)pl, counts, gg);
            if (t_planes == 2) {
                hipLaunchKernelGGL(h2_scale_from_absmax_kernel, dim3(1), dim3(256), 0, s, (const float*)nullptr, (int64_t)0, (const unsigned*)(counts + 6), (float*)(counts + 4));
                sc_dev = (const float*)(counts + 4);
            }
        } else {
            (void)hipMemsetAsync(counts, 0, 8 * sizeof(int), s);
            hipLaunchKernelGGL(sdf_mlp_active_points_kernel, dim3((unsigned)d3h_cdiv(n, 256)), dim3(256), 0, s, gout, n, pl, counts);
            if (t_planes == 2) {
                hipLaunchKernelGGL(h2_scale_from_absmax_kernel, dim3(1), dim3(256), 0, s, (const float*)nullptr, (int64_t)0, (const unsigned*)(counts + 2), (float*)(counts + 4));
                sc_dev = (const float*)(counts + 4);
            }
            hipLaunchKernelGGL(sdf_mlp_gather_points_kernel, dim3(256), dim3(256), 0, s, x, deform, disp, gout, (const int*)pl, counts, ident, xg, gg);
        }
        list = ident;
        cnt = counts + 1;
        xs = xg; dfs = nullptr; disps = 0.f; gs = gg; dxs = dx ? dxg : nullptr;
        plist = pl; pcounts = counts;
        if (!prepared) {
            int e = d3h_sdf_mlp_fwd_x3_list_launch(xs, nullptr, 0.f, wpack3_recompute, recompute_planes, (float*)act, n, list, cnt, s);
            if (e != 0) return e;
        }
    } else
#endif
    if (tile_list) {
        int nt16r = (int)((n + 15) / 16);
        int* count = tile_list + nt16r;
        (void)hipMemsetAsync(count, 0, sizeof(int), s);
        if (dx) (void)hipMemsetAsync(dx, 0, (size_t)n * 3 * sizeof(float), s);
        hipLaunchKernelGGL(sdf_mlp_active_tiles_kernel, dim3(d3h_cdiv(nt16r, 256)), dim3(256), 0, s, gout, n, nt16r, tile_list, count);
        list = tile_list;
        cnt = count;
    }
#if D3H_MLP_NOUT == 1
    if (wpack3_recompute && !tile_list) {
        int e = (recompute_planes == 2 ? d3h_sdf_mlp_fwd_h2 : d3h_sdf_mlp_fwd_x3)(x, deform, disp, wpack3_recompute, dz , nullptr, (float*)act, n, 0, s);
        if (e != 0) return e;
    }
#else
    if (wpack3_recompute) return D3H_ERR_ARG;
#endif
#if D3H_MLP_NOUT == 1
    if (wpackT3 && t_planes == 2 && !sc_dev) {
        if (hipMallocAsync((void**)&sc_tmp, 2 * sizeof(float), s) != hipSuccess) return D3H_ERR_ARG;
        hipLaunchKernelGGL(h2_scale_from_absmax_kernel, dim3(1), dim3(256), 0, s, gs, n * NOUT, (const unsigned*)nullptr, sc_tmp);
        sc_dev = sc_tmp;
    }
#endif
    const int ktb = d3h_ktime_begin(tile_list ? D3H_KT_SDF_BWD_DATA_SPARSE : D3H_KT_SDF_BWD_DATA, n, s);
#if D3H_MLP_NOUT == 1
    if (wpackT3)
        bwd_data_x_launch<false>(t_planes, grid, s, xs, dfs, disps, gs, w7, wpackT3, act, dz, dxs, n, ntiles, list, cnt, sc_dev, 1.0f);
    else
#endif
        hipLaunchKernelGGL((sdf_mlp_bwd_data_kernel<false>), dim3(grid), dim3(NTHREADS), 0, s, xs, dfs, disps, gs, w7, wpackT, act, dz, dxs, n,
                           ntiles, list, cnt);
    d3h_ktime_end(ktb, s);
#if D3H_MLP_NOUT == 1
    if (plist && dx) hipLaunchKernelGGL(sdf_mlp_scatter_dx_kernel, dim3(64), dim3(256), 0, s, (const float*)dxs, plist, pcounts, dx);
#endif
    int S = dw_split(nt32, DW_SPLIT);
    const int SE = dw_split(nt32, D3H_DW_SPLIT_EMB);
    const int SL = tile_list ? (nt32 < D3H_DW_SPLIT_SPARSE ? nt32 : D3H_DW_SPLIT_SPARSE) : S;
    const int SEL = (plist && SE > D3H_DW_SPLIT_SPARSE) ? D3H_DW_SPLIT_SPARSE : SE;
    const float* nof = nullptr;
    const int ktw = d3h_ktime_begin(D3H_KT_SDF_DW_LAYERS_SPARSE, n, s);
#if D3H_MLP_NOUT == 1
    if (wpackT3 && dw_x3_enabled(2))
    {
        if (t_planes == 2 && dw_h2_enabled())
            hipLaunchKernelGGL(sdf_mlp_bwd_dw_layers_h2_kernel, dim3(SL, 2, 6), dim3(512), 0, s, dz, act, nt16, dwh, dbh, dw4, db4, list, cnt, nof, nof, sc_dev, 1.0f, 1);
        else
            hipLaunchKernelGGL(sdf_mlp_bwd_dw_layers_x3_kernel, dim3(SL, 2, 6), dim3(512), 0, s, dz, act, nt16, dwh, dbh, dw4, db4, list, cnt, nof, nof);
    }
    else
#endif
        hipLaunchKernelGGL(sdf_mlp_bwd_dw_layers_kernel, dim3(SL, 2, 6), dim3(512), 0, s, dz, act, xs, n, nt32, dwh, dbh, dw4, db4, list, cnt, nof, nof);
    d3h_ktime_end(ktw, s);
    {
        const DwEmbArgs e4 = {dz + (size_t)4 * ACT_LAYER_FLOATS, act + (size_t)3 * ACT_LAYER_FLOATS, dw4, 256 + EMB_DIM, 256, EMB_DIM, (float*)nullptr, nof, nof, nof};
        const DwEmbArgs e0 = {dz, act, dw0, EMB_DIM, 0, EMB_DIM, db0, nof, nof, nof};
        hipLaunchKernelGGL(sdf_mlp_bwd_dw_emb_pair_kernel, dim3(SEL, 1, 2), dim3(512), 0, s, e4, e0, xs, dfs, disps, n, nt32, list, cnt);
    }
    int g7 = nt16 < LAST_GRID ? nt16 : LAST_GRID;
    hipLaunchKernelGGL(sdf_mlp_bwd_last_kernel, dim3(g7, NOUT), dim3(256), 0, s, gs, act + (size_t)6 * ACT_LAYER_FLOATS, n, nt16, dw7, db7, list, cnt);
    if (sc_tmp) (void)hipFreeAsync(sc_tmp, s);
    D3H_LAUNCH_CHECK();
    return D3H_OK;
}

#if D3H_MLP_NOUT == 1
int d3h_sdf_mlp_jvp_launch(const float* x, const float* udir, const float* wpack, const float* act, const float* dz, float* tb, float* eb,
                           int64_t n, int max_cus, hipStream_t s);
int d3h_sdf_mlp_jvp_x3_launch(const float* x, const float* udir, const unsigned* wpack3, int planes, float uscale, const float* act, const float* dz, float* tb,
                              float* eb, int64_t n, int max_cus, hipStream_t s);

extern "C" int d3h_sdf_mlp_grad_x(const float* x, const float* w7, const float* wpackT, const unsigned* wpackT3, int t_planes, const float* act, float* dz,
                                  int64_t n, float* g, int max_cus, void* stream) {
    if (n < 0) return D3H_ERR_ARG;
    if (wpackT3 && t_planes != 2 && t_planes != 3) return D3H_ERR_ARG;
    if (n == 0) return D3H_OK;
    if (!x || !w7 || (!wpackT && !wpackT3) || !act || !dz || !g) return D3H_ERR_ARG;
    int ntiles = (int)((n + TILE_PTS - 1) / TILE_PTS);
    int grid = sdf_chain_grid(ntiles, max_cus);
    const int kt = d3h_ktime_begin(D3H_KT_SDF_BWD_DATA, n, (hipStream_t)stream);
    if (wpackT3)
        bwd_data_x_launch<false>(t_planes, grid, (hipStream_t)stream, x, nullptr, 0.f, nullptr, w7, wpackT3, act, dz, g, n, ntiles, nullptr, nullptr, nullptr,
                                 h2_grad_scale(1.0f));
    else
        hipLaunchKernelGGL((sdf_mlp_bwd_data_kernel<false>), dim3(grid), dim3(NTHREADS), 0, (hipStream_t)stream, x, (const float*)nullptr, 0.f,
                           (const float*)nullptr, w7, wpackT, act, dz, g, n, ntiles, (const int*)nullptr, (const int*)nullptr);
    d3h_ktime_end(kt, (hipStream_t)stream);
    D3H_LAUNCH_CHECK();
    return D3H_OK;
}

extern "C" int d3h_eikonal_loss(const float* g, int64_t n, float scale, float* loss_sum, float* u, void* stream) {
    if (n < 0 || !loss_sum || (n > 0 && !g)) return D3H_ERR_ARG;
    hipStream_t s = (hipStream_t)stream;
    (void)hipMemsetAsync(loss_sum, 0, sizeof(float), s);
    if (n > 0) hipLaunchKernelGGL(eikonal_loss_kernel, dim3(d3h_grid(n, 256)), dim3(256), 0, s, g, n, scale, loss_sum, u);
    D3H_LAUNCH_CHECK();
    return D3H_OK;
}

extern "C" int d3h_sdf_mlp_eik_bwd(const float* x, const float* udir, const float* wpack, const float* wpackT, const unsigned* wpack3, int f_planes,
                                   const unsigned* wpackT3, int t_planes, float u_hint, const float* act,
                                   const float* dz, float* tb, float* eb, int64_t n, float* dw0, float* db0, float* dwh, float* dbh,
                                   float* dw4, float* db4, float* dw7, int max_cus, void* stream) {
    if (n < 0) return D3H_ERR_ARG;
    if (n == 0) return D3H_OK;
    if (!x || !udir || (!wpack && !wpack3) || (!wpackT && !wpackT3) || !act || !dz || !tb || !eb || !dw0 || !db0 || !dwh || !dbh || !dw4 || !db4 || !dw7)
        return D3H_ERR_ARG;
    if (wpackT3 && (t_planes != 2 && t_planes != 3)) return D3H_ERR_ARG;
    if (wpackT3 && t_planes == 2 && !(u_hint > 0.f)) return D3H_ERR_ARG;
    if (wpack3 && (f_planes != 2 && f_planes != 3)) return D3H_ERR_ARG;
    if (wpack3 && f_planes == 2 && !(u_hint > 0.f)) return D3H_ERR_ARG;
    hipStream_t s = (hipStream_t)stream;
    int ntiles = (int)((n + TILE_PTS - 1) / TILE_PTS);
    int nt32 = ntiles * 4;
    int grid = sdf_chain_grid(ntiles, max_cus);
    {
        int e = wpack3 ? d3h_sdf_mlp_jvp_x3_launch(x, udir, wpack3, f_planes, f_planes == 2 ? h2_grad_scale(u_hint * 256.0f) : 1.0f, act, dz, tb, eb, n, max_cus, s)
                       : d3h_sdf_mlp_jvp_launch(x, udir, wpack, act, dz, tb, eb, n, max_cus, s);
        if (e != 0) return e;
    }
    const int kti = d3h_ktime_begin(D3H_KT_SDF_BWD_INJECT, n, s);
    if (wpackT3)
        bwd_data_x_launch<true>(t_planes, grid, s, x, nullptr, 0.f, nullptr, (const float*)wpackT3, wpackT3, act, eb, nullptr, n, ntiles, nullptr, nullptr, nullptr,
                                h2_grad_scale(u_hint * 256.0f));
    else
        hipLaunchKernelGGL((sdf_mlp_bwd_data_kernel<true>), dim3(grid), dim3(NTHREADS), 0, s, x, (const float*)nullptr, 0.f, (const float*)nullptr,
                           wpackT, wpackT, act, eb, (float*)nullptr, n, ntiles, (const int*)nullptr, (const int*)nullptr);
    d3h_ktime_end(kti, s);
    int S = dw_split(nt32, DW_SPLIT);
    const int SE = dw_split(nt32, D3H_DW_SPLIT_EMB);
    const float* nof = nullptr;
    float* nob = nullptr;
    const int* noi = nullptr;
    const int ktd = d3h_ktime_begin(D3H_KT_SDF_DW_LAYERS, n, s);
    if (wpackT3 && dw_x3_enabled(3)) {
        int Sx = S;
        static int env_s = -1;
        if (env_s < 0) { const char* e = getenv("D3H_DWX_DUAL_SPLIT"); env_s = e ? atoi(e) : 0; }
        if (env_s > 0) Sx = env_s;
        else if (max_cus > 0 && max_cus <= 160 && max_cus / 12 >= 1 && max_cus / 12 < Sx) Sx = max_cus / 12;
        if (t_planes == 2 && dw_h2_enabled())
            hipLaunchKernelGGL(sdf_mlp_bwd_dw_layers_h2_kernel, dim3(Sx, 2, 6), dim3(512), 0, s, dz, tb, ntiles * 8, dwh, dbh, dw4, db4, noi, noi,
                               (const float*)eb, act, nof, h2_grad_scale(u_hint * 256.0f), 2 | 4);
        else
            hipLaunchKernelGGL(sdf_mlp_bwd_dw_layers_x3_kernel, dim3(Sx, 2, 6), dim3(512), 0, s, dz, tb, ntiles * 8, dwh, dbh, dw4, db4, noi, noi,
                               (const float*)eb, act);
    }
    else
        hipLaunchKernelGGL(sdf_mlp_bwd_dw_layers_kernel, dim3(S, 2, 6), dim3(512), 0, s, dz, tb, x, n, nt32, dwh, dbh, dw4, db4, noi, noi, (const float*)eb,
                           act);
    d3h_ktime_end(ktd, s);
    {
        const DwEmbArgs e4 = {dz + (size_t)4 * ACT_LAYER_FLOATS, tb + (size_t)3 * ACT_LAYER_FLOATS, dw4, 256 + EMB_DIM, 256, EMB_DIM, nob, udir,
                              (const float*)(eb + (size_t)4 * ACT_LAYER_FLOATS), act + (size_t)3 * ACT_LAYER_FLOATS};
        const DwEmbArgs e0 = {dz, act, dw0, EMB_DIM, 0, EMB_DIM, db0, udir, (const float*)eb, act};
        hipLaunchKernelGGL(sdf_mlp_bwd_dw_emb_pair_kernel, dim3(SE, 1, 2), dim3(512), 0, s, e4, e0, x, nof, 0.f, n, nt32, noi, noi);
    }
    int nt16 = ntiles * 8;
    int g7 = nt16 < LAST_GRID ? nt16 : LAST_GRID;
    hipLaunchKernelGGL(sdf_mlp_bwd_last_kernel, dim3(g7), dim3(256), 0, s, nof, tb + (size_t)6 * ACT_LAYER_FLOATS, n, nt16, dw7, nob, noi, noi);
    D3H_LAUNCH_CHECK();
    return D3H_OK;
}
#endif
```

d3human-code_amd/csrc/sdf_mlp_x3.hip:

```cpp
#include "sdf_mlp_dev.h"
#include "sdf_mlp_x3.h"

#if D3H_MLP_NOUT == 1

using namespace D3H_MLP_NS;

template <int NP>
__global__ void sdf_mlp_pack3_kernel(const float* __restrict__ w0, const float* __restrict__ b0, const float* __restrict__ wh,
                                     const float* __restrict__ bh, const float* __restrict__ w4, const float* __restrict__ b4,
                                     const float* __restrict__ w7, const float* __restrict__ b7, unsigned* __restrict__ wpack3) {
    int idx = blockIdx.x * blockDim.x + threadIdx.x;
    if (idx >= XP<NP>::WPACK_DWORDS) return;
    if (idx >= XP<NP>::OFF_TAIL) {
        int j = idx - XP<NP>::OFF_TAIL;
        float v = 0.f;
        if (j < 256) v = b0[j];
        else if (j < 256 * 7) {
            int l = j >> 8, f = j & 255;
            if (l == 4) v = b4[f];
            else v = bh[((l < 4) ? (l - 1) : (l - 2)) * 256 + f];
        } else if (j < HEAD_B) v = w7[j - HEAD_W];
        else if (j < HEAD_B + NOUT) v = b7[j - HEAD_B];
        wpack3[idx] = __float_as_uint(v);
        return;
    }
    const int l = XP<NP>::layer_of_offset(idx);
    const int local = idx - XP<NP>::layer_offset(l);
    const int d = local & 3, lane = (local >> 2) & 63;
    int rest = local >> 8;
    const int part = rest % NP;
    rest /= NP;
    const int nkb = (l == 0) ? X3_EMB_KB : ((l == 4) ? X3_SKIP_KB : 8);
    const int kb = rest % nkb, rbg = rest / nkb;
    const int i = lane & 15, q = lane >> 4;
    const int out = 16 * rbg + i;
    unsigned bits[2];
#pragma unroll
    for (int e = 0; e < 2; ++e) {
        const int s = 2 * d + e;
        float v = 0.f;
        if (l == 0) {
            const int in = x3_feature(kb, q, s);
            if (in < EMB_DIM) v = w0[out * EMB_DIM + in];
        } else if (l == 4) {
            if (kb < 8) v = w4[out * (256 + EMB_DIM) + x3_feature(kb, q, s)];
            else {
                const int in = x3_feature(kb - 8, q, s);
                if (in < EMB_DIM) v = w4[out * (256 + EMB_DIM) + 256 + in];
            }
        } else {
            const int hi = (l < 4) ? (l - 1) : (l - 2);
            v = wh[(size_t)hi * 65536 + out * 256 + x3_feature(kb, q, s)];
        }
        unsigned h, m, lo = 0;
        if constexpr (NP == 3) x3_split_pair(v, 0.f, h, m, lo);
        else {
            h2_split_pair(v, 0.f, h, m);
            if (!(fabsf(v) <= 16384.0f)) h = m = 0x7e00u;
        }
        bits[e] = (part == 0 ? h : (part == 1 ? m : lo)) & 0xffffu;
    }
    wpack3[idx] = bits[0] | (bits[1] << 16);
}

namespace {

__device__ __forceinline__ void x3_epilogue(f32x4& v, const float* bias_l, int rb, int lane, float* act_tile_layer) {
#ifdef D3H_X3_PROBE_NOEPI
    return;
#endif
    f32x4 b = *(const f32x4*)(bias_l + 16 * rb + 4 * (lane >> 4));
    f32x4 o;
#pragma unroll
    for (int r = 0; r < 4; ++r) {
        o[r] = softplus100(v[r] + b[r]);
        v[r] = o[r];
    }
    if (act_tile_layer) __builtin_nontemporal_store(o, (f32x4*)(act_tile_layer + (rb * 64 + lane) * 4));
}

__device__ __forceinline__ void x3_epilogue_jvp(f32x4& v, const f32x4 hh, const f32x4 dd, float* t_l, float* e_l, int rb, int lane, float usi) {
    const size_t off = (size_t)(rb * 64 + lane) * 4;
    f32x4 to, eo;
#pragma unroll
    for (int r = 0; r < 4; ++r) {
        const float sg = dsoftplus_from_h(hh[r]);
        const float qv = v[r];
        v[r] = sg * qv;
        to[r] = v[r] * usi;
        eo[r] = 100.0f * (1.0f - sg) * dd[r] * (qv * usi);
    }
    *(f32x4*)(t_l + off) = to;
    *(f32x4*)(e_l + off) = eo;
}

}

template <bool JVP, int SMALL, bool SAVE, int NP>
__global__ __launch_bounds__(NTHREADS, 2) void sdf_mlp_fwd_x3_kernel(const float* __restrict__ x, const float* __restrict__ deform, float disp,
                                                                    const unsigned* __restrict__ wpack3, float* __restrict__ sdf,
                                                                    float* __restrict__ xdef, float* __restrict__ act, int64_t n, int ntiles,
                                                                    const float* __restrict__ udir, const float* __restrict__ dzb,
                                                                    float* __restrict__ tb, float* __restrict__ eb,
                                                                    const int* __restrict__ tile_list, const int* __restrict__ tile_count, float uscale) {
    using P = XP<NP>;
    const float us = (JVP && NP == 2) ? uscale : 1.0f, usi = (JVP && NP == 2) ? 1.0f / uscale : 1.0f;
    __shared__ __attribute__((aligned(16))) unsigned wbuf[2][P::CHUNK_MAX];
    __shared__ __attribute__((aligned(16))) float bias[JVP ? 4 : BIAS_FLOATS];
    __shared__ __attribute__((aligned(16))) float jpf[JVP ? NWAVES * 4 * 256 : 4];

    D3H_X3_CLAIM_SIMD();
    const int tid = threadIdx.x;
    const int lane = tid & 63;
    const int wave = __builtin_amdgcn_readfirstlane(tid >> 6);
    const int q = lane >> 4;

    if (!JVP)
        for (int i = tid; i < BIAS_FLOATS; i += NTHREADS) bias[i] = __uint_as_float(wpack3[P::OFF_TAIL + i]);

    int pb = 0;
    x3_issue(wpack3, wbuf[0], P::L0_CHUNK / 4, tid);
    glds_commit();

    u32x4 Xs[8][NP];
    f32x4 Y[16];

    constexpr bool BAL = JVP || SMALL != 0 || NWAVES != 8;
    const int64_t n16 = (BAL && tile_list) ? (int64_t)*tile_count : (int64_t)ntiles * 8;
    const int G = (int)gridDim.x;
    const int nrounds = BAL ? (int)((n16 + NWAVES * (int64_t)G - 1) / (NWAVES * (int64_t)G)) : (ntiles - (int)blockIdx.x + G - 1) / G;
    for (int rnd = 0; rnd < nrounds; ++rnd) {
        const int tile = (int)blockIdx.x + rnd * G;
        int64_t t16 = BAL ? ((int64_t)rnd * NWAVES * G + (int64_t)wave * G + blockIdx.x) : ((int64_t)tile * 8 + wave);
        const bool on = !BAL || t16 < n16;
        if (BAL && tile_list) t16 = on ? (int64_t)tile_list[t16] : 0;
        const int64_t p = t16 * 16 + (lane & 15);
        const bool valid = p < n;
        float* act_tile = (SAVE || JVP) ? act + t16 * ACT_TILE_FLOATS : nullptr;
        const float* dz_tile = JVP ? dzb + t16 * ACT_TILE_FLOATS : nullptr;
        float* t_tile = JVP ? tb + t16 * ACT_TILE_FLOATS : nullptr;
        float* e_tile = JVP ? eb + t16 * ACT_TILE_FLOATS : nullptr;

        float x0 = 0.f, x1 = 0.f, x2 = 0.f;
        if (valid) {
            x0 = x[3 * p + 0]; x1 = x[3 * p + 1]; x2 = x[3 * p + 2];
            if (deform) {
                x0 = __fadd_rn(x0, __fmul_rn(disp, deform[3 * p + 0]));
                x1 = __fadd_rn(x1, __fmul_rn(disp, deform[3 * p + 1]));
                x2 = __fadd_rn(x2, __fmul_rn(disp, deform[3 * p + 2]));
            }
            if (xdef && q == 0) { xdef[3 * p + 0] = x0; xdef[3 * p + 1] = x1; xdef[3 * p + 2] = x2; }
        }
        u32x4 E3[X3_EMB_KB][NP];
        {
            float u0 = 0.f, u1 = 0.f, u2 = 0.f;
            if (JVP && valid) { u0 = udir[3 * p + 0] * us; u1 = udir[3 * p + 1] * us; u2 = udir[3 * p + 2] * us; }
#pragma unroll
            for (int kb = 0; kb < X3_EMB_KB; ++kb) {
                f32x4 v0, v1;
#pragma unroll
                for (int r = 0; r < 4; ++r) {
                    const int e0 = 32 * kb + 4 * q + r, e1 = e0 + 16;
                    v0[r] = JVP ? emb_tangent(e0, x0, x1, x2, u0, u1, u2) : emb_feature(e0, x0, x1, x2);
                    v1[r] = JVP ? emb_tangent(e1, x0, x1, x2, u0, u1, u2) : emb_feature(e1, x0, x1, x2);
                }
                xp_split_blocks<NP>(v0, v1, E3[kb]);
            }
        }

#pragma unroll
        for (int c = 0; c < 2; ++c) {
            const unsigned* nsrc = (c == 0) ? wpack3 + P::L0_CHUNK : wpack3 + P::OFF_L1;
            const int nn4 = ((c == 0) ? P::L0_CHUNK : P::HID_CHUNK) / 4;
            x3_issue(nsrc, wbuf[pb ^ 1], nn4, tid);
            const unsigned* wl = wbuf[pb];
            if (on) {
#pragma unroll
                for (int rbl = 0; rbl < 8; ++rbl) {
                    f32x4 acc = {0.f, 0.f, 0.f, 0.f}, lo = {0.f, 0.f, 0.f, 0.f};
                    xp_mac_blocks<NP, X3_EMB_KB, -1>(acc, lo, E3, wl + rbl * (X3_EMB_KB * NP * X3_FRAG), lane, X3None());
                    Y[8 * c + rbl] = xp_fold<NP>(acc, lo);
                }
            }
            glds_commit();
            pb ^= 1;
            if (on) {
#pragma unroll
                for (int rbl = 0; rbl < 8; ++rbl) {
                    const int rb = 8 * c + rbl;
                    if (JVP) {
                        const size_t off = (size_t)(rb * 64 + lane) * 4;
                        x3_epilogue_jvp(Y[rb], *(const f32x4*)(act_tile + off), *(const f32x4*)(dz_tile + off), t_tile, e_tile, rb, lane, usi);
                    } else x3_epilogue(Y[rb], bias, rb, lane, act_tile);
                }
            }
        }
#pragma unroll
        for (int kb = 0; kb < 8; ++kb) xp_split_blocks<NP>(Y[2 * kb], Y[2 * kb + 1], Xs[kb]);

        const bool late = !JVP && NWAVES == 8 && wave >= 4;
        auto epi = [&](f32x4& v, int l, int rb) { x3_epilogue(v, bias + 256 * l, rb, lane, act_tile ? act_tile + l * ACT_LAYER_FLOATS : nullptr); };
#pragma unroll 1
        for (int l = 1; l <= 6; ++l) {
            const bool skip = (l == 4);
            const int this_chunk = skip ? P::SKIP_CHUNK : P::HID_CHUNK;
            const int rstride = (skip ? X3_SKIP_KB : 8) * NP * X3_FRAG;
            const unsigned* lbase = wpack3 + P::layer_offset(l);
#pragma unroll
            for (int c = 0; c < 8; ++c) {
                const unsigned* nsrc = (c < 7) ? lbase + (c + 1) * this_chunk : ((l == 6) ? wpack3 : wpack3 + P::layer_offset(l + 1));
                const int nn4 = ((c < 7) ? this_chunk : ((l == 6) ? P::L0_CHUNK : ((l == 3) ? P::SKIP_CHUNK : P::HID_CHUNK))) / 4;
                x3_issue(nsrc, wbuf[pb ^ 1], nn4, tid);
                if (JVP && on) {
                    float* pf = jpf + wave * (4 * 256);
                    const size_t o0 = (size_t)l * ACT_LAYER_FLOATS + (size_t)((2 * c) * 64 + lane) * 4;
                    D3H_GLDS16(act_tile + o0, pf);
                    D3H_GLDS16(dz_tile + o0, pf + 256);
                    D3H_GLDS16(act_tile + o0 + 256, pf + 512);
                    D3H_GLDS16(dz_tile + o0 + 256, pf + 768);
                }
                const unsigned* wl = wbuf[pb];
                if (on) {
                    f32x4 acc0 = {0.f, 0.f, 0.f, 0.f}, acc1 = {0.f, 0.f, 0.f, 0.f}, lo0 = {0.f, 0.f, 0.f, 0.f}, lo1 = {0.f, 0.f, 0.f, 0.f};
                    xp_mac_blocks<NP, 8, 4>(acc0, lo0, Xs, wl, lane, [&] {
                        if (late) {
                            if (c > 0) { epi(Y[2 * c - 2], l, 2 * c - 2); epi(Y[2 * c - 1], l, 2 * c - 1); }
                            else if (l > 1) {
                                epi(Y[14], l - 1, 14);
                                epi(Y[15], l - 1, 15);
                                xp_split_blocks<NP>(Y[14], Y[15], Xs[7]);
                            }
                        }
                    });
#ifndef D3H_X3_PROBE_NOSKIP
                    if (skip) xp_mac_blocks<NP, X3_EMB_KB, -1>(acc0, lo0, E3, wl + 8 * NP * X3_FRAG, lane, X3None());
#endif
                    xp_mac_blocks<NP, 8, -1>(acc1, lo1, Xs, wl + rstride, lane, X3None());
#ifndef D3H_X3_PROBE_NOSKIP
                    if (skip) xp_mac_blocks<NP, X3_EMB_KB, -1>(acc1, lo1, E3, wl + rstride + 8 * NP * X3_FRAG, lane, X3None());
#endif
                    Y[2 * c] = xp_fold<NP>(acc0, lo0);
                    Y[2 * c + 1] = xp_fold<NP>(acc1, lo1);
                }
                glds_commit();
                pb ^= 1;
                if (JVP) {
                    if (on) {
                        const float* pf = jpf + wave * (4 * 256) + lane * 4;
                        float* tl = t_tile + l * ACT_LAYER_FLOATS;
                        float* el = e_tile + l * ACT_LAYER_FLOATS;
                        x3_epilogue_jvp(Y[2 * c], *(const f32x4*)pf, *(const f32x4*)(pf + 256), tl, el, 2 * c, lane, usi);
                        x3_epilogue_jvp(Y[2 * c + 1], *(const f32x4*)(pf + 512), *(const f32x4*)(pf + 768), tl, el, 2 * c + 1, lane, usi);
                    }
                } else if (on && !late) { epi(Y[2 * c], l, 2 * c); epi(Y[2 * c + 1], l, 2 * c + 1); }
            }
            if (l < 6) {
#pragma unroll
                for (int kb = 0; kb < 7; ++kb) xp_split_blocks<NP>(Y[2 * kb], Y[2 * kb + 1], Xs[kb]);
                if (!late) xp_split_blocks<NP>(Y[14], Y[15], Xs[7]);
            }
        }
        if (on && late) { epi(Y[14], 6, 14); epi(Y[15], 6, 15); }

        if (JVP || !on) continue;
#pragma unroll
        for (int o = 0; o < NOUT; ++o) {
            float part = 0.f;
#pragma unroll
            for (int rb = 0; rb < 16; ++rb) {
                f32x4 w = *(const f32x4*)(bias + HEAD_W + 256 * o + 16 * rb + 4 * q);
#pragma unroll
                for (int r = 0; r < 4; ++r) part = fmaf(w[r], Y[rb][r], part);
            }
            part += __shfl_xor(part, 16);
            part += __shfl_xor(part, 32);
            float tot = part + bias[HEAD_B + o];
            if (sdf && valid && q == 0) sdf[p * NOUT + o] = tot;
        }
    }
#if !defined(D3H_EMULATED)
    __builtin_amdgcn_s_waitcnt(0x0f70);
#endif
}

extern "C" int64_t d3h_sdf_mlp_wpack3_dwords(void) { return X3_WPACK_DWORDS; }

extern "C" int d3h_sdf_mlp_pack3(const float* w0, const float* b0, const float* wh, const float* bh, const float* w4, const float* b4,
                                 const float* w7, const float* b7, unsigned* wpack3, void* stream) {
    if (!w0 || !b0 || !wh || !bh || !w4 || !b4 || !w7 || !b7 || !wpack3) return D3H_ERR_ARG;
    hipLaunchKernelGGL(sdf_mlp_pack3_kernel<3>, dim3(d3h_cdiv(X3_WPACK_DWORDS, 256)), dim3(256), 0, (hipStream_t)stream, w0, b0, wh, bh, w4, b4, w7,
                       b7, wpack3);
    D3H_LAUNCH_CHECK();
    return D3H_OK;
}

extern "C" int64_t d3h_sdf_mlp_wpackh2_dwords(void) { return XP<2>::WPACK_DWORDS; }

extern "C" int d3h_sdf_mlp_pack_h2(const float* w0, const float* b0, const float* wh, const float* bh, const float* w4, const float* b4,
                                   const float* w7, const float* b7, unsigned* wpackh2, void* stream) {
    if (!w0 || !b0 || !wh || !bh || !w4 || !b4 || !w7 || !b7 || !wpackh2) return D3H_ERR_ARG;
    hipLaunchKernelGGL(sdf_mlp_pack3_kernel<2>, dim3(d3h_cdiv(XP<2>::WPACK_DWORDS, 256)), dim3(256), 0, (hipStream_t)stream, w0, b0, wh, bh, w4, b4,
                       w7, b7, wpackh2);
    D3H_LAUNCH_CHECK();
    return D3H_OK;
}

template <int NP>
static int fwd_xp_launch(const float* x, const float* deform, float disp, const unsigned* wpack, float* sdf, float* xdef, float* act, int64_t n, int max_cus,
                         void* stream) {
    if (n < 0 || (n > 0 && (!x || !wpack || !sdf))) return D3H_ERR_ARG;
    if (n == 0) return D3H_OK;
    int ntiles = (int)((n + TILE_PTS - 1) / TILE_PTS);
    int grid = sdf_chain_grid(ntiles, max_cus);
    const int kt = d3h_ktime_begin(D3H_KT_SDF_FWD, n, (hipStream_t)stream);
#define X3_FWD(SMALL_, SAVE_)                                                                                                                          \
    hipLaunchKernelGGL((sdf_mlp_fwd_x3_kernel<false, SMALL_, SAVE_, NP>), dim3(grid), dim3(NTHREADS), 0, (hipStream_t)stream, x, deform, disp, wpack, sdf, \
                       xdef, act, n, ntiles, (const float*)nullptr, (const float*)nullptr, (float*)nullptr, (float*)nullptr, (const int*)nullptr,          \
                       (const int*)nullptr, 1.0f)
    if (ntiles >= 1024) {
        if (act) X3_FWD(0, true); else X3_FWD(0, false);
    } else {
        if (act) X3_FWD(1, true); else X3_FWD(1, false);
    }
#undef X3_FWD
    d3h_ktime_end(kt, (hipStream_t)stream);
    D3H_LAUNCH_CHECK();
    return D3H_OK;
}

extern "C" int d3h_sdf_mlp_fwd_x3(const float* x, const float* deform, float disp, const unsigned* wpack3, float* sdf, float* xdef, float* act,
                                  int64_t n, int max_cus, void* stream) {
    return fwd_xp_launch<3>(x, deform, disp, wpack3, sdf, xdef, act, n, max_cus, stream);
}

extern "C" int d3h_sdf_mlp_fwd_h2(const float* x, const float* deform, float disp, const unsigned* wpackh2, float* sdf, float* xdef, float* act,
                                  int64_t n, int max_cus, void* stream) {
    return fwd_xp_launch<2>(x, deform, disp, wpackh2, sdf, xdef, act, n, max_cus, stream);
}

int d3h_sdf_mlp_jvp_x3_launch(const float* x, const float* udir, const unsigned* wpack3, int planes, float uscale, const float* act, const float* dz, float* tb,
                              float* eb, int64_t n, int max_cus, hipStream_t s) {
    int ntiles = (int)((n + TILE_PTS - 1) / TILE_PTS);
    int grid = sdf_chain_grid(ntiles, max_cus);
    const int kt = d3h_ktime_begin(D3H_KT_SDF_TANGENT, n, s);
    if (planes == 2)
        hipLaunchKernelGGL((sdf_mlp_fwd_x3_kernel<true, 1, false, 2>), dim3(grid), dim3(NTHREADS), 0, s, x, (const float*)nullptr, 0.f, wpack3, (float*)nullptr,
                           (float*)nullptr, (float*)act, n, ntiles, udir, dz, tb, eb, (const int*)nullptr, (const int*)nullptr, uscale);
    else
    hipLaunchKernelGGL((sdf_mlp_fwd_x3_kernel<true, 1, false, 3>), dim3(grid), dim3(NTHREADS), 0, s, x, (const float*)nullptr, 0.f, wpack3, (float*)nullptr,
                       (float*)nullptr, (float*)act, n, ntiles, udir, dz, tb, eb, (const int*)nullptr, (const int*)nullptr, 1.0f);
    d3h_ktime_end(kt, s);
    return (int)hipGetLastError();
}

int d3h_sdf_mlp_fwd_x3_list_launch(const float* x, const float* deform, float disp, const unsigned* wpack3, int planes, float* act, int64_t n,
                                   const int* tile_list, const int* tile_count, hipStream_t s) {
    int ntiles = (int)((n + TILE_PTS - 1) / TILE_PTS);
    int grid = sdf_chain_grid(ntiles, 0);
    const int kt = d3h_ktime_begin(D3H_KT_SDF_FWD_RECOMPUTE, n, s);
    if (planes == 2)
        hipLaunchKernelGGL((sdf_mlp_fwd_x3_kernel<false, 1, true, 2>), dim3(grid), dim3(NTHREADS), 0, s, x, deform, disp, wpack3, (float*)nullptr,
                           (float*)nullptr, act, n, ntiles, (const float*)nullptr, (const float*)nullptr, (float*)nullptr, (float*)nullptr, tile_list, tile_count, 1.0f);
    else
    hipLaunchKernelGGL((sdf_mlp_fwd_x3_kernel<false, 1, true, 3>), dim3(grid), dim3(NTHREADS), 0, s, x, deform, disp, wpack3, (float*)nullptr, (float*)nullptr,
                       act, n, ntiles, (const float*)nullptr, (const float*)nullptr, (float*)nullptr, (float*)nullptr, tile_list, tile_count, 1.0f);
    d3h_ktime_end(kt, s);
    return (int)hipGetLastError();
}

#endif
```

Measured before the change: 235.6.

## Store raw tangent q in JVP sweep and form eikonal inject terms downstream

The tangent (JVP) kernel gains a q-store mode. It writes the pre-activation tangent q instead of computing the e term from dz, and it accumulates the last-layer weight gradient (dw7) through per-wave shared sums plus atomics. This removes the separate bwd_last kernel. The inject backward kernel now computes e on the fly from dz, q and h, and the dw-layer kernel rebuilds dsoftplus*q pairwise using interleaved tile ordering. This cuts dz reads and e writes in the JVP sweep and drops a kernel launch. In exchange the inject kernel prefetches more data, the atomics make dw7 accumulation order nondeterministic, and an extra __syncthreads is added.

```diff
diff --git a/d3human-code_amd/csrc/sdf_mlp_bwd.hip b/d3human-code_amd/csrc/sdf_mlp_bwd.hip
--- a/d3human-code_amd/csrc/sdf_mlp_bwd.hip
+++ b/d3human-code_amd/csrc/sdf_mlp_bwd.hip
@@ -444,19 +444,29 @@
     *(f32x4*)(e_l + (size_t)(rb * 64 + lane) * 4) = o;
 }
 
-template <bool INJECT, int NP>
+__device__ __forceinline__ f32x4 e_from_q(const f32x4 hh, const f32x4 dd, const f32x4 qq) {
+    f32x4 e;
+#pragma unroll
+    for (int r = 0; r < 4; ++r) e[r] = 100.0f * (1.0f - dsoftplus_from_h(hh[r])) * dd[r] * qq[r];
+    return e;
+}
+
+template <bool INJECT, int NP, bool QIN = false>
 __global__ __launch_bounds__(NTHREADS, 2) void sdf_mlp_bwd_data_x3_kernel(const float* __restrict__ x, const float* __restrict__ deform, float disp,
                                                                          const float* __restrict__ gout, const float* __restrict__ w7,
                                                                          const unsigned* __restrict__ wpackT3, const float* __restrict__ act,
                                                                          float* __restrict__ dz, float* __restrict__ dx, int64_t n, int ntiles,
                                                                          const int* __restrict__ tile_list, const int* __restrict__ tile_count,
-                                                                         const float* __restrict__ sc_dev, float sc_imm) {
+                                                                         const float* __restrict__ sc_dev, float sc_imm, const float* __restrict__ dzin,
+                                                                         const float* __restrict__ qb) {
+    static_assert(!QIN || INJECT, "QIN forms the injected term");
     constexpr int X3_HID_CHUNK = XPT<NP>::HID_CHUNK;
     const float gs = (NP == 2) ? (sc_dev ? sc_dev[0] : sc_imm) : 1.0f;
     const float gsi = (NP == 2) ? (sc_dev ? sc_dev[1] : 1.0f / sc_imm) : 1.0f;
     __shared__ __attribute__((aligned(16))) unsigned wbuf[2][X3_HID_CHUNK];
     __shared__ __attribute__((aligned(16))) float w7s[NOUT * 256];
-    __shared__ __attribute__((aligned(16))) float pfb[NWAVES * (INJECT ? 4 : 2) * 256];
+    constexpr int PFW = (QIN ? 6 : (INJECT ? 4 : 2)) * 256;
+    __shared__ __attribute__((aligned(16))) float pfb[NWAVES * PFW];
     D3H_X3_CLAIM_SIMD();
     const int n_active = tile_list ? *tile_count : 0;
     const int64_t n16 = tile_list ? (int64_t)n_active : (int64_t)ntiles * 8;
@@ -486,6 +496,8 @@
         const bool valid = on && p < n;
         const float* act_tile = act + t16 * ACT_TILE_FLOATS;
         float* dz_tile = dz + t16 * ACT_TILE_FLOATS;
+        const float* dzin_tile = QIN ? dzin + t16 * ACT_TILE_FLOATS : nullptr;
+        const float* q_tile = QIN ? qb + t16 * ACT_TILE_FLOATS : nullptr;
         float g[NOUT];
 #pragma unroll
         for (int o = 0; o < NOUT; ++o) g[o] = INJECT ? 0.f : (valid ? (gout ? gout[p * NOUT + o] : 1.f) * gs : 0.f);
@@ -502,7 +514,9 @@
             if (on) {
                 const size_t off6 = (size_t)6 * ACT_LAYER_FLOATS + (size_t)(rb * 64 + lane) * 4;
                 const f32x4 hh6 = *(const f32x4*)(act_tile + off6);
-                if (INJECT) dzs_inject<NP == 2>(Y[rb], hh6, *(const f32x4*)(dz_tile + off6), dz_tile + 6 * ACT_LAYER_FLOATS, rb, lane, gs, gsi);
+                if (QIN) dzs_inject<NP == 2>(Y[rb], hh6, e_from_q(hh6, *(const f32x4*)(dzin_tile + off6), *(const f32x4*)(q_tile + off6)),
+                                             dz_tile + 6 * ACT_LAYER_FLOATS, rb, lane, gs, gsi);
+                else if (INJECT) dzs_inject<NP == 2>(Y[rb], hh6, *(const f32x4*)(dz_tile + off6), dz_tile + 6 * ACT_LAYER_FLOATS, rb, lane, gs, gsi);
                 else dzs_plain<NP == 2>(Y[rb], hh6, dz_tile + 6 * ACT_LAYER_FLOATS, rb, lane, gsi);
             }
         }
@@ -513,12 +527,17 @@
 #pragma unroll
         for (int b = 0; b < 4; ++b) E[b] = Elo[b] = (f32x4){0.f, 0.f, 0.f, 0.f};
 
-        float* pf = pfb + wave * ((INJECT ? 4 : 2) * 256);
+        float* pf = pfb + wave * PFW;
         auto prefetch = [&](int lp, int c) {
             const size_t o0 = (size_t)lp * ACT_LAYER_FLOATS + (size_t)((2 * c) * 64 + lane) * 4;
             D3H_GLDS16(act_tile + o0, pf);
             D3H_GLDS16(act_tile + o0 + 256, pf + 256);
-            if (INJECT) {
+            if (QIN) {
+                D3H_GLDS16(dzin_tile + o0, pf + 512);
+                D3H_GLDS16(dzin_tile + o0 + 256, pf + 768);
+                D3H_GLDS16(q_tile + o0, pf + 1024);
+                D3H_GLDS16(q_tile + o0 + 256, pf + 1280);
+            } else if (INJECT) {
                 D3H_GLDS16(dz_tile + o0, pf + 512);
                 D3H_GLDS16(dz_tile + o0 + 256, pf + 768);
             }
@@ -526,7 +545,11 @@
         auto dz_pair = [&](f32x4& v0, f32x4& v1, int lp, int c) {
             const float* pl = pf + lane * 4;
             float* dzl = dz_tile + lp * ACT_LAYER_FLOATS;
-            if (INJECT) {
+            if (QIN) {
+                const f32x4 h0 = *(const f32x4*)pl, h1 = *(const f32x4*)(pl + 256);
+                dzs_inject<NP == 2>(v0, h0, e_from_q(h0, *(const f32x4*)(pl + 512), *(const f32x4*)(pl + 1024)), dzl, 2 * c, lane, gs, gsi);
+                dzs_inject<NP == 2>(v1, h1, e_from_q(h1, *(const f32x4*)(pl + 768), *(const f32x4*)(pl + 1280)), dzl, 2 * c + 1, lane, gs, gsi);
+            } else if (INJECT) {
                 dzs_inject<NP == 2>(v0, *(const f32x4*)pl, *(const f32x4*)(pl + 512), dzl, 2 * c, lane, gs, gsi);
                 dzs_inject<NP == 2>(v1, *(const f32x4*)(pl + 256), *(const f32x4*)(pl + 768), dzl, 2 * c + 1, lane, gs, gsi);
             } else {
@@ -629,13 +652,17 @@
 template <bool INJECT>
 static inline void bwd_data_x_launch(int planes, int grid, hipStream_t s, const float* x, const float* deform, float disp, const float* gout, const float* w7,
                                      const unsigned* wpackT, const float* act, float* dz, float* dx, int64_t n, int ntiles, const int* list, const int* cnt,
-                                     const float* sc_dev, float sc_imm) {
-    if (planes == 2)
+                                     const float* sc_dev, float sc_imm, const float* dzin = nullptr, const float* qb = nullptr) {
+    const float* nof = nullptr;
+    if (INJECT && qb && planes == 2)
+        hipLaunchKernelGGL((sdf_mlp_bwd_data_x3_kernel<INJECT, 2, INJECT>), dim3(grid), dim3(NTHREADS), 0, s, x, deform, disp, gout, w7, wpackT, act, dz, dx, n,
+                           ntiles, list, cnt, sc_dev, sc_imm, dzin, qb);
+    else if (planes == 2)
         hipLaunchKernelGGL((sdf_mlp_bwd_data_x3_kernel<INJECT, 2>), dim3(grid), dim3(NTHREADS), 0, s, x, deform, disp, gout, w7, wpackT, act, dz, dx, n, ntiles,
-                           list, cnt, sc_dev, sc_imm);
+                           list, cnt, sc_dev, sc_imm, nof, nof);
     else
         hipLaunchKernelGGL((sdf_mlp_bwd_data_x3_kernel<INJECT, 3>), dim3(grid), dim3(NTHREADS), 0, s, x, deform, disp, gout, w7, wpackT, act, dz, dx, n, ntiles,
-                           list, cnt, (const float*)nullptr, 1.0f);
+                           list, cnt, (const float*)nullptr, 1.0f, nof, nof);
 }
 #endif
 
@@ -1101,7 +1128,7 @@
                                                                        float* __restrict__ db4, const int* __restrict__ tile_list,
                                                                        const int* __restrict__ tile_count, const float* __restrict__ a2_base,
                                                                        const float* __restrict__ b2_base, const float* __restrict__ sc_dev, float sc_imm,
-                                                                       int sc_mask) {
+                                                                       int sc_mask, int qpair) {
     __shared__ __attribute__((aligned(16))) unsigned TAs[2][2 * 256 * DWX_PITCH];
     __shared__ __attribute__((aligned(16))) unsigned TBs[2][2 * 128 * DWX_PITCH];
     D3H_X3_CLAIM_SIMD();
@@ -1133,6 +1160,7 @@
     }
     const int n16 = tile_list ? *tile_count : ntiles16;
     const int ngroups = dz2 ? 2 * n16 : n16;
+    const bool qp = dz2 && qpair;
     const int G2 = 2 * (int)gridDim.x;
     int t = 2 * (int)blockIdx.x;
     if (t >= ngroups) return;
@@ -1140,8 +1168,8 @@
     f32x4 ra[2][2], rb[2];
     float sca[2], scb[2];
     auto issue = [&](int slot, int tv) {
-        const bool second = dz2 && tv >= n16;
-        const int tt = second ? tv - n16 : tv;
+        const bool second = qp ? (tv & 1) != 0 : (dz2 && tv >= n16);
+        const int tt = qp ? tv >> 1 : (second ? tv - n16 : tv);
         const int64_t tl = tile_list ? (int64_t)tile_list[tt] : (int64_t)tt;
         const float* __restrict__ asrc = (second ? dz2 : dz_l) + (size_t)tl * ACT_TILE_FLOATS;
         const float* __restrict__ bsrc = (second ? hsrc2 : hsrc) + (size_t)tl * ACT_TILE_FLOATS;
@@ -1156,6 +1184,10 @@
     if (t + 1 < ngroups) issue(1, t + 1);
     for (; t < ngroups; t += G2) {
         const bool two = t + 1 < ngroups;
+        if (qp) {
+#pragma unroll
+            for (int r = 0; r < 4; ++r) rb[0][r] = dsoftplus_from_h(rb[1][r]) * rb[0][r];
+        }
 #pragma unroll
         for (int sl = 0; sl < 2; ++sl) {
             if (sl == 1 && !two) break;
@@ -1163,8 +1195,8 @@
             dwh_put(TAs[sl], 256, 16 * (wave + 8) + 4 * (lane >> 4), lane & 15, ra[sl][1], sca[sl]);
             dwh_put(TBs[sl], 128, 16 * wave + 4 * (lane >> 4), lane & 15, rb[sl], scb[sl]);
         }
-        const bool bias0 = want_db && db && (!dz2 || t >= n16);
-        const bool bias1 = want_db && db && two && (!dz2 || t + 1 >= n16);
+        const bool bias0 = want_db && db && (!dz2 || (!qp && t >= n16));
+        const bool bias1 = want_db && db && two && (!dz2 || qp || t + 1 >= n16);
         __syncthreads();
         if (t + G2 < ngroups) {
             issue(0, t + G2);
@@ -1200,6 +1232,7 @@
         }
         __syncthreads();
     }
+    __syncthreads();
     const float wsc = gsi * (1.0f / DWH_US);
     const bool a_flag = dz2 ? ((sc_mask >> 2) & 1) : (sc_mask & 1);
     const float bsc = a_flag ? gsi : (1.0f / DWH_US);
@@ -1464,7 +1497,7 @@
     if (wpackT3 && dw_x3_enabled(2))
     {
         if (t_planes == 2 && dw_h2_enabled())
-            hipLaunchKernelGGL(sdf_mlp_bwd_dw_layers_h2_kernel, dim3(SL, 2, 6), dim3(512), 0, s, dz, act, nt16, dwh, dbh, dw4, db4, list, cnt, nof, nof, sc_dev, 1.0f, 1);
+            hipLaunchKernelGGL(sdf_mlp_bwd_dw_layers_h2_kernel, dim3(SL, 2, 6), dim3(512), 0, s, dz, act, nt16, dwh, dbh, dw4, db4, list, cnt, nof, nof, sc_dev, 1.0f, 1, 0);
         else
             hipLaunchKernelGGL(sdf_mlp_bwd_dw_layers_x3_kernel, dim3(SL, 2, 6), dim3(512), 0, s, dz, act, nt16, dwh, dbh, dw4, db4, list, cnt, nof, nof);
     }
@@ -1488,7 +1521,12 @@
 int d3h_sdf_mlp_jvp_launch(const float* x, const float* udir, const float* wpack, const float* act, const float* dz, float* tb, float* eb,
                            int64_t n, int max_cus, hipStream_t s);
 int d3h_sdf_mlp_jvp_x3_launch(const float* x, const float* udir, const unsigned* wpack3, int planes, float uscale, const float* act, const float* dz, float* tb,
-                              float* eb, int64_t n, int max_cus, hipStream_t s);
+                              float* eb, float* dw7, int64_t n, int max_cus, hipStream_t s);
+
+static inline bool eik_qstore_enabled() {
+    const char* e = getenv("D3H_EIK_QSTORE");
+    return !(e && e[0] == '0');
+}
 
 extern "C" int d3h_sdf_mlp_grad_x(const float* x, const float* w7, const float* wpackT, const unsigned* wpackT3, int t_planes, const float* act, float* dz,
                                   int64_t n, float* g, int max_cus, void* stream) {
@@ -1535,15 +1573,18 @@
     int ntiles = (int)((n + TILE_PTS - 1) / TILE_PTS);
     int nt32 = ntiles * 4;
     int grid = sdf_chain_grid(ntiles, max_cus);
+    const bool qstore = wpack3 && f_planes == 2 && wpackT3 && t_planes == 2 && dw_x3_enabled(3) && dw_h2_enabled() && eik_qstore_enabled();
     {
-        int e = wpack3 ? d3h_sdf_mlp_jvp_x3_launch(x, udir, wpack3, f_planes, f_planes == 2 ? h2_grad_scale(u_hint * 256.0f) : 1.0f, act, dz, tb, eb, n, max_cus, s)
+        int e = wpack3 ? d3h_sdf_mlp_jvp_x3_launch(x, udir, wpack3, f_planes, f_planes == 2 ? h2_grad_scale(u_hint * 256.0f) : 1.0f, act, dz, tb, eb,
+                                                   qstore ? dw7 : nullptr, n, max_cus, s)
                        : d3h_sdf_mlp_jvp_launch(x, udir, wpack, act, dz, tb, eb, n, max_cus, s);
         if (e != 0) return e;
     }
     const int kti = d3h_ktime_begin(D3H_KT_SDF_BWD_INJECT, n, s);
     if (wpackT3)
         bwd_data_x_launch<true>(t_planes, grid, s, x, nullptr, 0.f, nullptr, (const float*)wpackT3, wpackT3, act, eb, nullptr, n, ntiles, nullptr, nullptr, nullptr,
-                                h2_grad_scale(u_hint * 256.0f));
+                                h2_grad_scale(u_hint * 256.0f),
+                                qstore ? dz : nullptr, qstore ? tb : nullptr);
     else
         hipLaunchKernelGGL((sdf_mlp_bwd_data_kernel<true>), dim3(grid), dim3(NTHREADS), 0, s, x, (const float*)nullptr, 0.f, (const float*)nullptr,
                            wpackT, wpackT, act, eb, (float*)nullptr, n, ntiles, (const int*)nullptr, (const int*)nullptr);
@@ -1562,7 +1603,7 @@
         else if (max_cus > 0 && max_cus <= 160 && max_cus / 12 >= 1 && max_cus / 12 < Sx) Sx = max_cus / 12;
         if (t_planes == 2 && dw_h2_enabled())
             hipLaunchKernelGGL(sdf_mlp_bwd_dw_layers_h2_kernel, dim3(Sx, 2, 6), dim3(512), 0, s, dz, tb, ntiles * 8, dwh, dbh, dw4, db4, noi, noi,
-                               (const float*)eb, act, nof, h2_grad_scale(u_hint * 256.0f), 2 | 4);
+                               (const float*)eb, act, nof, h2_grad_scale(u_hint * 256.0f), 2 | 4, qstore ? 1 : 0);
         else
             hipLaunchKernelGGL(sdf_mlp_bwd_dw_layers_x3_kernel, dim3(Sx, 2, 6), dim3(512), 0, s, dz, tb, ntiles * 8, dwh, dbh, dw4, db4, noi, noi,
                                (const float*)eb, act);
@@ -1577,9 +1618,11 @@
         const DwEmbArgs e0 = {dz, act, dw0, EMB_DIM, 0, EMB_DIM, db0, udir, (const float*)eb, act};
         hipLaunchKernelGGL(sdf_mlp_bwd_dw_emb_pair_kernel, dim3(SE, 1, 2), dim3(512), 0, s, e4, e0, x, nof, 0.f, n, nt32, noi, noi);
     }
-    int nt16 = ntiles * 8;
-    int g7 = nt16 < LAST_GRID ? nt16 : LAST_GRID;
-    hipLaunchKernelGGL(sdf_mlp_bwd_last_kernel, dim3(g7), dim3(256), 0, s, nof, tb + (size_t)6 * ACT_LAYER_FLOATS, n, nt16, dw7, nob, noi, noi);
+    if (!qstore) {
+        int nt16 = ntiles * 8;
+        int g7 = nt16 < LAST_GRID ? nt16 : LAST_GRID;
+        hipLaunchKernelGGL(sdf_mlp_bwd_last_kernel, dim3(g7), dim3(256), 0, s, nof, tb + (size_t)6 * ACT_LAYER_FLOATS, n, nt16, dw7, nob, noi, noi);
+    }
     D3H_LAUNCH_CHECK();
     return D3H_OK;
 }
diff --git a/d3human-code_amd/csrc/sdf_mlp_x3.hip b/d3human-code_amd/csrc/sdf_mlp_x3.hip
--- a/d3human-code_amd/csrc/sdf_mlp_x3.hip
+++ b/d3human-code_amd/csrc/sdf_mlp_x3.hip
@@ -93,21 +93,34 @@
     *(f32x4*)(t_l + off) = to;
     *(f32x4*)(e_l + off) = eo;
 }
-
-}
-
-template <bool JVP, int SMALL, bool SAVE, int NP>
+__device__ __forceinline__ void x3_epilogue_jvp_q(f32x4& v, const f32x4 hh, float* q_l, int rb, int lane, float usi) {
+    f32x4 qo;
+#pragma unroll
+    for (int r = 0; r < 4; ++r) {
+        const float qv = v[r];
+        v[r] = dsoftplus_from_h(hh[r]) * qv;
+        qo[r] = qv * usi;
+    }
+    *(f32x4*)(q_l + (size_t)(rb * 64 + lane) * 4) = qo;
+}
+
+}
+
+template <bool JVP, int SMALL, bool SAVE, int NP, bool QS = false>
 __global__ __launch_bounds__(NTHREADS, 2) void sdf_mlp_fwd_x3_kernel(const float* __restrict__ x, const float* __restrict__ deform, float disp,
                                                                     const unsigned* __restrict__ wpack3, float* __restrict__ sdf,
                                                                     float* __restrict__ xdef, float* __restrict__ act, int64_t n, int ntiles,
                                                                     const float* __restrict__ udir, const float* __restrict__ dzb,
                                                                     float* __restrict__ tb, float* __restrict__ eb,
-                                                                    const int* __restrict__ tile_list, const int* __restrict__ tile_count, float uscale) {
+                                                                    const int* __restrict__ tile_list, const int* __restrict__ tile_count, float uscale,
+                                                                    float* __restrict__ dw7) {
+    static_assert(!QS || JVP, "the q-store layout is a tangent-sweep layout");
     using P = XP<NP>;
     const float us = (JVP && NP == 2) ? uscale : 1.0f, usi = (JVP && NP == 2) ? 1.0f / uscale : 1.0f;
     __shared__ __attribute__((aligned(16))) unsigned wbuf[2][P::CHUNK_MAX];
     __shared__ __attribute__((aligned(16))) float bias[JVP ? 4 : BIAS_FLOATS];
     __shared__ __attribute__((aligned(16))) float jpf[JVP ? NWAVES * 4 * 256 : 4];
+    __shared__ __attribute__((aligned(16))) float t6sum[QS ? NWAVES * 256 : 4];
 
     D3H_X3_CLAIM_SIMD();
     const int tid = threadIdx.x;
@@ -117,6 +130,9 @@
 
     if (!JVP)
         for (int i = tid; i < BIAS_FLOATS; i += NTHREADS) bias[i] = __uint_as_float(wpack3[P::OFF_TAIL + i]);
+
+    if (QS)
+        for (int i = tid; i < NWAVES * 256; i += NTHREADS) t6sum[i] = 0.f;
 
     int pb = 0;
     x3_issue(wpack3, wbuf[0], P::L0_CHUNK / 4, tid);
@@ -137,9 +153,9 @@
         const int64_t p = t16 * 16 + (lane & 15);
         const bool valid = p < n;
         float* act_tile = (SAVE || JVP) ? act + t16 * ACT_TILE_FLOATS : nullptr;
-        const float* dz_tile = JVP ? dzb + t16 * ACT_TILE_FLOATS : nullptr;
+        const float* dz_tile = (JVP && !QS) ? dzb + t16 * ACT_TILE_FLOATS : nullptr;
         float* t_tile = JVP ? tb + t16 * ACT_TILE_FLOATS : nullptr;
-        float* e_tile = JVP ? eb + t16 * ACT_TILE_FLOATS : nullptr;
+        float* e_tile = (JVP && !QS) ? eb + t16 * ACT_TILE_FLOATS : nullptr;
 
         float x0 = 0.f, x1 = 0.f, x2 = 0.f;
         if (valid) {
@@ -190,7 +206,8 @@
                     const int rb = 8 * c + rbl;
                     if (JVP) {
                         const size_t off = (size_t)(rb * 64 + lane) * 4;
-                        x3_epilogue_jvp(Y[rb], *(const f32x4*)(act_tile + off), *(const f32x4*)(dz_tile + off), t_tile, e_tile, rb, lane, usi);
+                        if (QS) x3_epilogue_jvp_q(Y[rb], *(const f32x4*)(act_tile + off), t_tile, rb, lane, usi);
+                        else x3_epilogue_jvp(Y[rb], *(const f32x4*)(act_tile + off), *(const f32x4*)(dz_tile + off), t_tile, e_tile, rb, lane, usi);
                     } else x3_epilogue(Y[rb], bias, rb, lane, act_tile);
                 }
             }
@@ -215,9 +232,9 @@
                     float* pf = jpf + wave * (4 * 256);
                     const size_t o0 = (size_t)l * ACT_LAYER_FLOATS + (size_t)((2 * c) * 64 + lane) * 4;
                     D3H_GLDS16(act_tile + o0, pf);
-                    D3H_GLDS16(dz_tile + o0, pf + 256);
+                    if (!QS) D3H_GLDS16(dz_tile + o0, pf + 256);
                     D3H_GLDS16(act_tile + o0 + 256, pf + 512);
-                    D3H_GLDS16(dz_tile + o0 + 256, pf + 768);
+                    if (!QS) D3H_GLDS16(dz_tile + o0 + 256, pf + 768);
                 }
                 const unsigned* wl = wbuf[pb];
                 if (on) {
@@ -248,9 +265,14 @@
                     if (on) {
                         const float* pf = jpf + wave * (4 * 256) + lane * 4;
                         float* tl = t_tile + l * ACT_LAYER_FLOATS;
-                        float* el = e_tile + l * ACT_LAYER_FLOATS;
-                        x3_epilogue_jvp(Y[2 * c], *(const f32x4*)pf, *(const f32x4*)(pf + 256), tl, el, 2 * c, lane, usi);
-                        x3_epilogue_jvp(Y[2 * c + 1], *(const f32x4*)(pf + 512), *(const f32x4*)(pf + 768), tl, el, 2 * c + 1, lane, usi);
+                        if (QS) {
+                            x3_epilogue_jvp_q(Y[2 * c], *(const f32x4*)pf, tl, 2 * c, lane, usi);
+                            x3_epilogue_jvp_q(Y[2 * c + 1], *(const f32x4*)(pf + 512), tl, 2 * c + 1, lane, usi);
+                        } else {
+                            float* el = e_tile + l * ACT_LAYER_FLOATS;
+                            x3_epilogue_jvp(Y[2 * c], *(const f32x4*)pf, *(const f32x4*)(pf + 256), tl, el, 2 * c, lane, usi);
+                            x3_epilogue_jvp(Y[2 * c + 1], *(const f32x4*)(pf + 512), *(const f32x4*)(pf + 768), tl, el, 2 * c + 1, lane, usi);
+                        }
                     }
                 } else if (on && !late) { epi(Y[2 * c], l, 2 * c); epi(Y[2 * c + 1], l, 2 * c + 1); }
             }
@@ -261,6 +283,20 @@
             }
         }
         if (on && late) { epi(Y[14], 6, 14); epi(Y[15], 6, 15); }
+        if (QS && on) {
+            float* ws = t6sum + wave * 256;
+#pragma unroll
+            for (int rb = 0; rb < 16; ++rb)
+#pragma unroll
+                for (int r = 0; r < 4; ++r) {
+                    float v = valid ? Y[rb][r] * usi : 0.f;
+                    v += __shfl_xor(v, 1);
+                    v += __shfl_xor(v, 2);
+                    v += __shfl_xor(v, 4);
+                    v += __shfl_xor(v, 8);
+                    if ((lane & 15) == 0) ws[16 * rb + 4 * q + r] += v;
+                }
+        }
 
         if (JVP || !on) continue;
 #pragma unroll
@@ -276,6 +312,15 @@
             part += __shfl_xor(part, 32);
             float tot = part + bias[HEAD_B + o];
             if (sdf && valid && q == 0) sdf[p * NOUT + o] = tot;
+        }
+    }
+    if (QS) {
+        __syncthreads();
+        if (tid < 256) {
+            float sm = 0.f;
+#pragma unroll
+            for (int w = 0; w < NWAVES; ++w) sm += t6sum[w * 256 + tid];
+            atomicAdd(dw7 + tid, sm);
         }
     }
 #if !defined(D3H_EMULATED)
@@ -316,7 +361,7 @@
 #define X3_FWD(SMALL_, SAVE_)                                                                                                                          \
     hipLaunchKernelGGL((sdf_mlp_fwd_x3_kernel<false, SMALL_, SAVE_, NP>), dim3(grid), dim3(NTHREADS), 0, (hipStream_t)stream, x, deform, disp, wpack, sdf, \
                        xdef, act, n, ntiles, (const float*)nullptr, (const float*)nullptr, (float*)nullptr, (float*)nullptr, (const int*)nullptr,          \
-                       (const int*)nullptr, 1.0f)
+                       (const int*)nullptr, 1.0f, (float*)nullptr)
     if (ntiles >= 1024) {
         if (act) X3_FWD(0, true); else X3_FWD(0, false);
     } else {
@@ -339,16 +384,21 @@
 }
 
 int d3h_sdf_mlp_jvp_x3_launch(const float* x, const float* udir, const unsigned* wpack3, int planes, float uscale, const float* act, const float* dz, float* tb,
-                              float* eb, int64_t n, int max_cus, hipStream_t s) {
+                              float* eb, float* dw7, int64_t n, int max_cus, hipStream_t s) {
+    if (dw7 && planes != 2) return D3H_ERR_ARG;
     int ntiles = (int)((n + TILE_PTS - 1) / TILE_PTS);
     int grid = sdf_chain_grid(ntiles, max_cus);
     const int kt = d3h_ktime_begin(D3H_KT_SDF_TANGENT, n, s);
-    if (planes == 2)
+    if (dw7)
+        hipLaunchKernelGGL((sdf_mlp_fwd_x3_kernel<true, 1, false, 2, true>), dim3(grid), dim3(NTHREADS), 0, s, x, (const float*)nullptr, 0.f, wpack3,
+                           (float*)nullptr, (float*)nullptr, (float*)act, n, ntiles, udir, (const float*)nullptr, tb, (float*)nullptr, (const int*)nullptr,
+                           (const int*)nullptr, uscale, dw7);
+    else if (planes == 2)
         hipLaunchKernelGGL((sdf_mlp_fwd_x3_kernel<true, 1, false, 2>), dim3(grid), dim3(NTHREADS), 0, s, x, (const float*)nullptr, 0.f, wpack3, (float*)nullptr,
-                           (float*)nullptr, (float*)act, n, ntiles, udir, dz, tb, eb, (const int*)nullptr, (const int*)nullptr, uscale);
+                           (float*)nullptr, (float*)act, n, ntiles, udir, dz, tb, eb, (const int*)nullptr, (const int*)nullptr, uscale, (float*)nullptr);
     else
     hipLaunchKernelGGL((sdf_mlp_fwd_x3_kernel<true, 1, false, 3>), dim3(grid), dim3(NTHREADS), 0, s, x, (const float*)nullptr, 0.f, wpack3, (float*)nullptr,
-                       (float*)nullptr, (float*)act, n, ntiles, udir, dz, tb, eb, (const int*)nullptr, (const int*)nullptr, 1.0f);
+                       (float*)nullptr, (float*)act, n, ntiles, udir, dz, tb, eb, (const int*)nullptr, (const int*)nullptr, 1.0f, (float*)nullptr);
     d3h_ktime_end(kt, s);
     return (int)hipGetLastError();
 }
@@ -360,10 +410,10 @@
     const int kt = d3h_ktime_begin(D3H_KT_SDF_FWD_RECOMPUTE, n, s);
     if (planes == 2)
         hipLaunchKernelGGL((sdf_mlp_fwd_x3_kernel<false, 1, true, 2>), dim3(grid), dim3(NTHREADS), 0, s, x, deform, disp, wpack3, (float*)nullptr,
-                           (float*)nullptr, act, n, ntiles, (const float*)nullptr, (const float*)nullptr, (float*)nullptr, (float*)nullptr, tile_list, tile_count, 1.0f);
+                           (float*)nullptr, act, n, ntiles, (const float*)nullptr, (const float*)nullptr, (float*)nullptr, (float*)nullptr, tile_list, tile_count, 1.0f, (float*)nullptr);
     else
     hipLaunchKernelGGL((sdf_mlp_fwd_x3_kernel<false, 1, true, 3>), dim3(grid), dim3(NTHREADS), 0, s, x, deform, disp, wpack3, (float*)nullptr, (float*)nullptr,
-                       act, n, ntiles, (const float*)nullptr, (const float*)nullptr, (float*)nullptr, (float*)nullptr, tile_list, tile_count, 1.0f);
+                       act, n, ntiles, (const float*)nullptr, (const float*)nullptr, (float*)nullptr, (float*)nullptr, tile_list, tile_count, 1.0f, (float*)nullptr);
     d3h_ktime_end(kt, s);
     return (int)hipGetLastError();
 }
```

After: 237.9, median of 6. No clear change (+1.0%).
